# zabaras/deep-turbulence

Measured on AMD Instinct MI355X. Metric: flow-field samples/sec (fwd+log-det+bwd), 64x256x256x4; optimizer step: HipAdam (one-launch Adam, same update as torch.optim.Adam), higher is better.
Workload: dtype f32; 1 GPU; tmglow M: sample()+logdet+backward+Adam, out 256x256x4, L=4, K=16, batch 64/GPU; global_batch=64, parallelism=dp1, world_size_observed=1, rank0_device=AMD Radeon Graphics cuda:0, mix_precision=f32, launch=eager

## Files before the change

deep-turbulence_amd/csrc/tmg_common.h:

```cpp
#pragma once
#include <hip/hip_runtime.h>
#include <stdint.h>
#include <stdlib.h>
#include <atomic>

typedef float f32x4 __attribute__((ext_vector_type(4)));

__device__ __forceinline__ __amdgpu_buffer_rsrc_t tmg_make_rsrc(const void* base, unsigned bytes) {
    return __builtin_amdgcn_make_buffer_rsrc(const_cast<void*>(base), 0, (int)bytes, 0x00020000);
}
__device__ __forceinline__ float4 tmg_bload4(__amdgpu_buffer_rsrc_t rs, unsigned voff, unsigned soff) {
    const f32x4 v = __builtin_bit_cast(f32x4, __builtin_amdgcn_raw_buffer_load_b128(rs, (int)voff, (int)soff, 0));
    return make_float4(v[0], v[1], v[2], v[3]);
}

#define TMG_MAX_IN_SEG 3
#define TMG_MAX_OUT_SEG 3

struct TmgSeg {
    const float* p;
    int stride;
    int off;
    int n;
};
struct TmgOSeg {
    float* p;
    int stride;
    int off;
    int n;
};

__device__ __forceinline__ float wave_sum(float v) {
#pragma unroll
    for (int o = 32; o > 0; o >>= 1) v += __shfl_xor(v, o, 64);
    return v;
}

__device__ __forceinline__ float block_sum_256(float v, float* red ) {
    v = wave_sum(v);
    const int lane = threadIdx.x & 63, w = threadIdx.x >> 6;
    __syncthreads();
    if (lane == 0) red[w] = v;
    __syncthreads();
    return red[0] + red[1] + red[2] + red[3];
}

__device__ __forceinline__ float out_scale_of(const float* kappa) {
    if (!kappa) return 1.0f;
    float k = *kappa;
    k = fminf(fmaxf(k, -4.0f), 1.3862943611198906f);
    return expf(k);
}

#define TMG_PICK_SEG(PTYPE_, ARR, C_, PTR_, STRIDE_, OFF_)                                                \
    PTYPE_ PTR_ = ARR[0].p;                                                                               \
    int STRIDE_ = ARR[0].stride, OFF_ = ARR[0].off;                                                       \
    if (C_ >= ARR[0].n) {                                                                                 \
        C_ -= ARR[0].n; PTR_ = ARR[1].p; STRIDE_ = ARR[1].stride; OFF_ = ARR[1].off;                      \
        if (C_ >= ARR[1].n) { C_ -= ARR[1].n; PTR_ = ARR[2].p; STRIDE_ = ARR[2].stride; OFF_ = ARR[2].off; } \
    }
#define TMG_PICK_OSEG(ARR, NL_, PTR_, STRIDE_, OFF_) TMG_PICK_SEG(float*, ARR, NL_, PTR_, STRIDE_, OFF_)

template <typename P>
__device__ __forceinline__ float4 load_in4(const P& p, int b, int iy, int ix, int c) {
    float4 v = make_float4(0.f, 0.f, 0.f, 0.f);
    if (p.pad_rep) {
        iy = min(max(iy, 0), p.Hin - 1);
        ix = min(max(ix, 0), p.Win - 1);
    } else if (iy < 0 || iy >= p.Hin || ix < 0 || ix >= p.Win) {
        return v;
    }
    if (c >= p.Cin) return v;
    const size_t pix = ((size_t)b * p.Hin + iy) * p.Win + ix;
    if (p.vec4) {
        int cl = c;
        TMG_PICK_SEG(const float*, p.in, cl, sp, ss, so)
        v = *reinterpret_cast<const float4*>(sp + pix * ss + so + cl);
    } else {
        float t[4];
#pragma unroll
        for (int e = 0; e < 4; ++e) {
            int cl = c + e;
            float x = 0.f;
            if (cl < p.Cin) {
                TMG_PICK_SEG(const float*, p.in, cl, sp, ss, so)
                x = sp[pix * ss + so + cl];
            }
            t[e] = x;
        }
        v = make_float4(t[0], t[1], t[2], t[3]);
    }
    if (p.in_scale) {
        float* f = reinterpret_cast<float*>(&v);
#pragma unroll
        for (int e = 0; e < 4; ++e)
            if (c + e < p.Cin) f[e] = f[e] * p.in_scale[c + e] + p.in_shift[c + e];
    }
    if (p.relu_in) {
        v.x = fmaxf(v.x, 0.f);
        v.y = fmaxf(v.y, 0.f);
// ... 248 lines not shown
```

deep-turbulence_amd/csrc/tmg_conv.hip:

```cpp
#include "tmg_common.h"
#include <stdlib.h>

static __device__ float g_tmg_zero_page[64];

struct ConvP {
    TmgSeg in[TMG_MAX_IN_SEG];
    int nseg;
    int vec4;
    int B, Hin, Win, Hout, Wout;
    int ksize, stride;
    int Cin, Cin_pad, Cout, Cout_pad;
    const float* wpk;
    const float* bias;
    const float* kappa;
    const float* in_scale;
    const float* in_shift;
    int relu_in, pad_rep, relu_out, accumulate;
    TmgOSeg out[TMG_MAX_OUT_SEG];
    int nout;
    TmgSeg add;
    int TW_log2, TH;
    int KCH;
    int tiles_x, tiles_y;
    int ntiles, nchunks;
// ... 808 lines not shown
        __syncthreads();
    }
#undef TMG_WG_MFMA
#undef TMG_SB
#undef TMG_WG_ISSUE
#undef TMG_WG_COMMIT
#undef TMG_WG_ISSUE_F
#undef TMG_WG_COMMIT_F
#undef TMG_WG_PATCH_ITEM
#undef TMG_WG_ORIGIN

    const int nws = ksplit ? 1 : 4;
    for (int half = 4; half >= nws; half >>= 1) {
        __syncthreads();
        if (wave >= half && wave < 2 * half) {
            float4* dst = reinterpret_cast<float4*>(lds) + ((wave - half) * NP * NCO) * 64 + lane;
#pragma unroll
            for (int j = 0; j < NP; ++j)
#pragma unroll
                for (int n = 0; n < NCO; ++n)
                    dst[(j * NCO + n) * 64] = make_float4(acc[j][n][0], acc[j][n][1], acc[j][n][2], acc[j][n][3]);
        }
        __syncthreads();
        if (wave < half) {
            const float4* src = reinterpret_cast<const float4*>(lds) + (wave * NP * NCO) * 64 + lane;
#pragma unroll
            for (int j = 0; j < NP; ++j)
#pragma unroll
                for (int n = 0; n < NCO; ++n) {
                    const float4 v = src[(j * NCO + n) * 64];
                    acc[j][n][0] += v.x; acc[j][n][1] += v.y; acc[j][n][2] += v.z; acc[j][n][3] += v.w;
                }
        }
    }
    float bsum = 0.f;
    const bool do_bias = p.dbias && blockIdx.z == 0;
    if (do_bias) {
        __syncthreads();
        *reinterpret_cast<float4*>(lds + tid * 4) = bacc;
        __syncthreads();
        if (tid < NCO * 16) {
            const int c4 = tid >> 2, e = tid & 3;
            for (int t = c4; t < NT; t += NCO * 4) bsum += lds[t * 4 + e];
        }
    }
    if (p.ws) {
        const size_t bl = ((size_t)blockIdx.x * gridDim.y + blockIdx.y) * gridDim.z + blockIdx.z;
        if (wave < nws) {
            float4* slab = reinterpret_cast<float4*>(p.ws) + ((bl * nws + wave) * NP * NCO) * 64 + lane;
#pragma unroll
            for (int j = 0; j < NP; ++j)
#pragma unroll
                for (int n = 0; n < NCO; ++n)
                    slab[(j * NCO + n) * 64] = make_float4(acc[j][n][0], acc[j][n][1], acc[j][n][2], acc[j][n][3]);
        }
        if (do_bias && tid < NCO * 16) {
            float* wsb = p.ws + (size_t)gridDim.x * gridDim.y * gridDim.z * nws * NP * NCO * 256;
            wsb[((size_t)blockIdx.x * gridDim.y + blockIdx.y) * 64 + tid] = bsum;
        }
        return;
    }
    if (wave >= nws) return;
    const float osc = out_scale_of(p.kappa);
#pragma unroll
    for (int j = 0; j < NP; ++j) {
        const int pid = ksplit ? j : w4 + 4 * j;
        if (pid >= npairs) continue;
        const int citg = (pair0 + pid) / ntaps, tap = pair0 + pid - citg * ntaps;
#pragma unroll
        for (int n = 0; n < NCO; ++n) {
            const int co = co0 + n * 16 + li;
            if (co >= p.Cout) continue;
#pragma unroll
            for (int r = 0; r < 4; ++r) {
                const int ci = citg * 16 + q * 4 + r;
                if (ci < p.cin_valid)
                    atomicAdd(p.dW + ((size_t)co * p.cin_dst + ci + (ci < p.ci_split ? p.ci_off0 : p.ci_off1)) * ntaps + tap, acc[j][n][r] * osc);
            }
        }
    }
    if (do_bias && tid < NCO * 16 && co0 + tid < p.Cout) atomicAdd(p.dbias + co0 + tid, bsum * osc);
}

__global__ void conv_wgrad_reduce_kernel(const float* __restrict__ ws, float* __restrict__ dW, float* __restrict__ dbias,
                                         const float* __restrict__ kappa, int gx, int gy, int gz, int NP, int NCO, int PPG,
                                         int pairs_total, int Cin, int Cout, int ntaps, int xchunk, int cin_valid, int ci_split,
                                         int ci_off0, int ci_off1, int ksplit, int bpg, long long dw_gstride, int db_gstride) {
    const int nws = ksplit ? 1 : 4;
    const int items = gy * gz * nws * NP * NCO * 64;
    const int i = blockIdx.x * blockDim.x + threadIdx.x;
    const int x0 = blockIdx.y * xchunk, x1 = min(gx, x0 + xchunk);
    const float osc = out_scale_of(kappa);
    if (i < items) {
        int r_ = i;
        const int lane = r_ & 63; r_ >>= 6;
        const int n = r_ % NCO; r_ /= NCO;
        const int j = r_ % NP; r_ /= NP;
        const int wave = r_ % nws; r_ /= nws;
        const int z = r_ % gz;
        const int y = r_ / gz;
        const int pid = ksplit ? j : wave + 4 * j;
        if (pid < min(PPG, pairs_total - z * PPG)) {
            const size_t per_x = (size_t)gy * gz * nws * NP * NCO * 64;
            const float4* src = reinterpret_cast<const float4*>(ws) + (((((size_t)y * gz + z) * nws + wave) * NP + j) * NCO + n) * 64 + lane;
            float4 a = make_float4(0.f, 0.f, 0.f, 0.f);
            for (int xb = x0; xb < x1; xb += 8) {
                float4 v[8];
#pragma unroll
                for (int u = 0; u < 8; ++u) v[u] = src[(size_t)min(xb + u, x1 - 1) * per_x];
#pragma unroll
                for (int u = 0; u < 8; ++u) {
                    const float wgt = (xb + u < x1) ? 1.f : 0.f;
                    a.x += wgt * v[u].x; a.y += wgt * v[u].y; a.z += wgt * v[u].z; a.w += wgt * v[u].w;
                }
            }
            const int citg = (z * PPG + pid) / ntaps, tap = z * PPG + pid - citg * ntaps;
            const int grp = y / bpg;
            const int co = ((y - grp * bpg) * NCO + n) * 16 + (lane & 15);
            const int ci = citg * 16 + (lane >> 4) * 4;
            dW += (size_t)grp * dw_gstride;
            if (co < Cout) {
                const float av[4] = {a.x, a.y, a.z, a.w};
#pragma unroll
                for (int r = 0; r < 4; ++r)
                    if (ci + r < cin_valid)
                        atomicAdd(dW + ((size_t)co * Cin + ci + r + (ci + r < ci_split ? ci_off0 : ci_off1)) * ntaps + tap, av[r] * osc);
            }
        }
    }
    if (dbias && i < gy * 64) {
        const int y = i >> 6, t = i & 63;
        const int grp = y / bpg;
        const int co = (y - grp * bpg) * NCO * 16 + t;
        dbias += (size_t)grp * db_gstride;
        if (t < NCO * 16 && co < Cout) {
            const float* wsb = ws + (size_t)gx * gy * gz * nws * NP * NCO * 256;
            float a = 0.f;
            for (int xb = x0; xb < x1; xb += 8) {
                float v[8];
#pragma unroll
                for (int u = 0; u < 8; ++u) v[u] = wsb[((size_t)min(xb + u, x1 - 1) * gy + y) * 64 + t];
#pragma unroll
                for (int u = 0; u < 8; ++u) a += (xb + u < x1) ? v[u] : 0.f;
            }
            atomicAdd(dbias + co, a * osc);
        }
    }
}

__global__ void conv_pack_kernel(const float* __restrict__ w, float* __restrict__ wpk, int Cout, int Cin, int ntaps,
                                 int Kpad, int Npad, int mode, int cvalid, int csplit, int cgap, size_t w_bstride, size_t wpk_bstride) {
    w += blockIdx.y * w_bstride;
    wpk += blockIdx.y * wpk_bstride;
    const size_t total = (size_t)ntaps * Kpad * Npad;
    for (size_t i = blockIdx.x * (size_t)blockDim.x + threadIdx.x; i < total; i += (size_t)gridDim.x * blockDim.x) {
        const int c16 = i & 15;
        size_t r = i >> 4;
        const int n = r % Npad;
        r /= Npad;
        const int kb = r % (Kpad >> 4);
        const int tap = r / (Kpad >> 4);
        const int k = kb * 16 + c16;
        float v = 0.f;
        if (mode == 0) {
            if (k < cvalid && n < Cout) v = w[((size_t)n * Cin + k + (k < csplit ? 0 : cgap)) * ntaps + tap];
        } else {
            if (k < Cout && n < cvalid) v = w[((size_t)k * Cin + n + (n < csplit ? 0 : cgap)) * ntaps + (ntaps - 1 - tap)];
        }
        wpk[i] = v;
    }
}

struct PackJob {
    const float* w; float* wpk;
    int Cout, Cin, ntaps, Kpad, Npad, mode, cvalid, csplit, cgap;
};
constexpr int TMG_PACK_JOBS = 48;
struct PackJobs { PackJob j[TMG_PACK_JOBS]; };

__global__ void conv_pack_many_kernel(PackJobs J) {
    const PackJob& jb = J.j[blockIdx.y];
    const float* __restrict__ w = jb.w;
    float* __restrict__ wpk = jb.wpk;
    const int Cout = jb.Cout, Cin = jb.Cin, ntaps = jb.ntaps, Kpad = jb.Kpad, Npad = jb.Npad, mode = jb.mode;
    const int cvalid = jb.cvalid, csplit = jb.csplit, cgap = jb.cgap;
    const size_t total = (size_t)ntaps * Kpad * Npad;
    for (size_t i = blockIdx.x * (size_t)blockDim.x + threadIdx.x; i < total; i += (size_t)gridDim.x * blockDim.x) {
        const int c16 = i & 15;
        size_t r = i >> 4;
        const int n = r % Npad;
        r /= Npad;
        const int kb = r % (Kpad >> 4);
        const int tap = r / (Kpad >> 4);
        const int k = kb * 16 + c16;
        float v = 0.f;
        if (mode == 0) {
            if (k < cvalid && n < Cout) v = w[((size_t)n * Cin + k + (k < csplit ? 0 : cgap)) * ntaps + tap];
        } else {
            if (k < Cout && n < cvalid) v = w[((size_t)k * Cin + n + (n < csplit ? 0 : cgap)) * ntaps + (ntaps - 1 - tap)];
        }
        wpk[i] = v;
    }
}

struct BorderP {
    const float* dy;
    int dy_stride, dy_off, Cdy;
    const float* wpk;
    int Cx, Npad, KB, dy_vec;
    const float* kappa;
    int B, H, W;
    TmgOSeg out[TMG_MAX_OUT_SEG];
    int nborder;
};

__device__ __forceinline__ void border_pixel(int idx, int H, int W, int* y, int* x) {
    if (idx < W) { *y = 0; *x = idx; return; }
    idx -= W;
    if (H > 1) {
        if (idx < W) { *y = H - 1; *x = idx; return; }
        idx -= W;
    }
    const int rows = H - 2;
    if (idx < rows) { *y = 1 + idx; *x = 0; return; }
    idx -= rows;
    *y = 1 + idx; *x = W - 1;
}

__global__ void conv_rep_border_fix_kernel(BorderP p) {
    const size_t total = (size_t)p.B * p.nborder * p.Cx;
// ... 576 lines not shown
    auto fits = [&](int cg, int nc) {
        if (cg > 8) return false;
        const int k4p = cg <= 1 ? 4 : (cg <= 2 ? 8 : (cg <= 4 ? 16 : 32));
        return PH * PW * k4p <= 7 * 512 && 2 * ((size_t)(PH * PW * 16 + 16) * cg + (size_t)(pl->MPIX * 16 + 16) * nc) * 4 <= 160 * 1024;
    };
    int CITG = 1, NCO = 1, bestg = -1;
    for (auto& c : pref) {
        int cg = c[0], nc = c[1];
        if (ntaps == 1) cg *= 4;
        if (cg > cit) {
            if (cit <= 2 && cot >= 8 && nc < 4 && ntaps == 9) continue;
            cg = cit;
        }
        if (nc > cot || (nc == 4 && !allow4)) continue;
        while (cg > 1 && !fits(cg, nc)) --cg;
        if (!fits(cg, nc)) continue;
        const int g = ((cit + cg - 1) / cg) * ((cot + nc - 1) / nc);
        if (g >= gmin) { CITG = cg; NCO = nc; bestg = g; break; }
        if (g > bestg) { CITG = cg; NCO = nc; bestg = g; }
    }
    if (bestg < 0) return -6;
    const int ngroups = (cit + CITG - 1) / CITG;
    pl->CITG = (cit + ngroups - 1) / ngroups;
    pl->NCO = NCO;
    pl->ksplit = ntaps * pl->CITG <= (NCO == 4 ? 5 : 9);
    pl->PPG = ntaps * pl->CITG;
    if (!pl->ksplit && ngroups > 1) {
        const int tp = ntaps * cit, ppg = (((tp + ngroups - 1) / ngroups) + 3) & ~3;
        int span = 0;
        for (int g = 0; g * ppg < tp; ++g) {
            const int a = g * ppg, b = (a + ppg < tp ? a + ppg : tp) - 1;
            if (b / ntaps - a / ntaps + 1 > span) span = b / ntaps - a / ntaps + 1;
        }
        if (ppg < pl->PPG && (ngroups - 1) * ppg < tp && span <= 4 && fits(span, NCO)) { pl->PPG = ppg; pl->CITG = span; }
    }
    const int np = pl->ksplit ? pl->PPG : (pl->PPG + 3) / 4;
    pl->NP = np <= 3 ? 3 : (np <= 5 ? 5 : (np <= 7 ? 7 : (np <= 8 ? 8 : 9)));
    if (pl->NP == 8 && NCO == 4) pl->NP = 9;
    if (np > 9) return -7;
    pl->gy = (cot + NCO - 1) / NCO;
    pl->gz = ngroups;
    int PHe = PH, PWe = PW;
    if (pl->ksplit && NCO == 1 && stride == 1 && TW >= 16 && pl->MPIX == 128) {
        const int k4p = pl->CITG <= 1 ? 4 : (pl->CITG <= 2 ? 8 : (pl->CITG <= 4 ? 16 : 32));
        for (int mp = 512; mp > 128; mp >>= 1) {
            const int th = mp >> twl, ph = th + 2 * halo;
            const int tiles = B * ((Wout + TW - 1) / TW) * ((Hout + th - 1) / th);
            if (ph * PW * k4p <= 7 * 512 && 2 * ((size_t)(ph * PW * 16 + 16) * pl->CITG + (size_t)(mp * 16 + 16) * NCO) * 4 <= 160 * 1024 &&
                tiles >= 4 * tmg_num_cus() / (pl->gy * pl->gz)) {
                pl->MPIX = mp; pl->TH = th;
                pl->tiles_y = (Hout + th - 1) / th;
                pl->ntiles = tiles;
                PHe = ph;
                break;
            }
        }
    }
    pl->lds_bytes = 2 * ((size_t)(PHe * PWe * 16 + 16) * pl->CITG + (size_t)(pl->MPIX * 16 + 16) * NCO) * 4;
    if (pl->lds_bytes < 8192) pl->lds_bytes = 8192;
    if (pl->lds_bytes < (size_t)4 * pl->NP * NCO * 1024) pl->lds_bytes = (size_t)4 * pl->NP * NCO * 1024;
    int gx = tmg_num_cus() / (pl->gy * ngroups);
    if (gx > pl->ntiles / 4) gx = pl->ntiles / 4;
    if (gx < 1) gx = 1;
    pl->gx = gx;
    pl->ws_floats = (size_t)gx * pl->gy * pl->gz * (pl->ksplit ? 1 : 4) * pl->NP * NCO * 256 + (size_t)gx * pl->gy * 64;
    return 0;
}

static int plan_wgrad(int B, int Hout, int Wout, int ksize, int stride, int Cin, int Cout, WgradPlan* pl) {
    const int rc = plan_wgrad_impl(B, Hout, Wout, ksize, stride, Cin, Cout, pl, true);
    if (rc == 0 && pl->NP == 5 && pl->NCO == 4) return plan_wgrad_impl(B, Hout, Wout, ksize, stride, Cin, Cout, pl, false);
    return rc;
}

extern "C" int64_t tmg_conv_wgrad_ws_floats(const int64_t* dims) {
    WgradPlan pl;
    if (plan_wgrad((int)dims[0], (int)dims[3], (int)dims[4], (int)dims[5], (int)dims[6], (int)dims[7], (int)dims[8], &pl) != 0) return 0;
    return (int64_t)pl.ws_floats;
}

static int wgrad_impl(const void* const* in_ptrs, const int64_t* in_desc, int64_t nseg, const void* in_scale,
                      const void* in_shift, const void* dy, const int64_t* dy_desc, void* dW, void* dbias,
                      const void* kappa, void* ws, int64_t ws_floats, const int64_t* dims, hipStream_t st,
                      const long long* gtab, int ngroups, int dy_goff, long long dw_gstride, int db_gstride, int64_t* plan = nullptr) {
    WgradP p;
    p.nseg = (int)nseg;
    p.vec4 = tmg_decode_in(p.in, in_ptrs, in_desc, nseg).vec4;
    p.B = (int)dims[0]; p.Hin = (int)dims[1]; p.Win = (int)dims[2]; p.Hout = (int)dims[3]; p.Wout = (int)dims[4];
    p.ksize = (int)dims[5]; p.stride = (int)dims[6]; p.Cin = (int)dims[7]; p.Cout = (int)dims[8];
    p.relu_in = (int)dims[9]; p.pad_rep = (int)dims[10];
    p.cin_dst = dims[11] > 0 ? (int)dims[11] : p.Cin;
    p.cin_valid = dims[12] > 0 ? (int)dims[12] : (p.cin_dst < p.Cin ? p.cin_dst : p.Cin);
    p.ci_split = dims[13] > 0 ? (int)dims[13] : 0x7fffffff;
    p.ci_off0 = (int)dims[14]; p.ci_off1 = (int)dims[15];
    if (p.ksize != 1 && p.ksize != 3) return -2;
    p.Cin_pad = (p.Cin + 15) & ~15;
    p.in_scale = (const float*)in_scale; p.in_shift = (const float*)in_shift;
    p.dy = TmgSeg{(const float*)dy, (int)dy_desc[0], (int)dy_desc[1], p.Cout};
    p.dy_vec4 = (((p.dy.stride | p.dy.off) & 3) == 0) && ((((uintptr_t)dy) & 15) == 0);
    p.dW = (float*)dW; p.dbias = (float*)dbias; p.kappa = (const float*)kappa;
    WgradPlan pl;
    const int rc = plan_wgrad(p.B, p.Hout, p.Wout, p.ksize, p.stride, p.Cin, p.Cout, &pl);
    if (rc != 0) return rc;
    p.TW_log2 = pl.twl; p.TH = pl.TH; p.MPIX = pl.MPIX; p.tiles_x = pl.tiles_x; p.tiles_y = pl.tiles_y; p.ntiles = pl.ntiles; p.CITG = pl.CITG;
    p.PPG = pl.PPG;
    const int bpg = pl.gy;
    if (ngroups > 1) {
        pl.gy = bpg * ngroups;
        int gx = tmg_num_cus() / (pl.gy * pl.gz);
        if (gx > pl.ntiles / 4) gx = pl.ntiles / 4;
        if (gx < 1) gx = 1;
        pl.gx = gx;
        pl.ws_floats = (size_t)gx * pl.gy * pl.gz * (pl.ksplit ? 1 : 4) * pl.NP * pl.NCO * 256 + (size_t)gx * pl.gy * 64;
    }
    p.ws = (ws && (size_t)ws_floats >= pl.ws_floats && (((uintptr_t)ws) & 15) == 0) ? (float*)ws : nullptr;
    dim3 grid(pl.gx, pl.gy, pl.gz);
    p.ksplit = pl.ksplit;
    p.gtab = gtab; p.bpg = bpg; p.dy_goff = dy_goff; p.dw_gstride = dw_gstride; p.db_gstride = db_gstride;
    p.fstage = p.vec4 && p.dy_vec4 && (p.Cout % 4 == 0) && (p.Cin % 4 == 0) && (long)p.Hin * p.Win < (1 << 24) && (long)p.Hout * p.Wout < (1 << 24);
    for (int i = 0; i < p.nseg; ++i)
        if (p.in[i].stride >= (1 << 24) || (long)p.B * p.Hin * p.Win * p.in[i].stride >= (1L << 31)) p.fstage = 0;
    if (p.dy.stride >= (1 << 24) || (long)p.B * p.Hout * p.Wout * p.dy.stride >= (1L << 31)) p.fstage = 0;
    if (ngroups > 1 && (!p.fstage || !p.ws)) return -100;
    int lrc = -7;
#define TMG_WG_CASE(NP_, NCO_)                                                                    \
    if (pl.NP == NP_ && pl.NCO == NCO_)                                                           \
        lrc = p.fstage ? launch_wgrad<NP_, NCO_, true>(p, grid, pl.lds_bytes, st, plan, pl.ws_floats)                       \
                       : launch_wgrad<NP_, NCO_, false>(p, grid, pl.lds_bytes, st, plan, pl.ws_floats);
    TMG_WG_CASE(3, 1) TMG_WG_CASE(3, 2) TMG_WG_CASE(3, 4)
    TMG_WG_CASE(5, 1) TMG_WG_CASE(5, 2)
    TMG_WG_CASE(7, 1) TMG_WG_CASE(7, 2)
    TMG_WG_CASE(8, 1) TMG_WG_CASE(8, 2)
    TMG_WG_CASE(9, 1) TMG_WG_CASE(9, 2)
#undef TMG_WG_CASE
    if (lrc != 0 || plan) return lrc;
    if (p.ws) {
        const int items = pl.gy * pl.gz * (pl.ksplit ? 1 : 4) * pl.NP * pl.NCO * 64;
        int xchunk = 32;
        const int xc = (pl.gx + xchunk - 1) / xchunk;
        hipLaunchKernelGGL(conv_wgrad_reduce_kernel, dim3((items + 255) / 256, xc), dim3(256), 0, st, (const float*)p.ws, p.dW, p.dbias,
                           p.kappa, pl.gx, pl.gy, pl.gz, pl.NP, pl.NCO, pl.PPG, (p.Cin_pad >> 4) * p.ksize * p.ksize, p.cin_dst, p.Cout, p.ksize * p.ksize, xchunk,
                           p.cin_valid, p.ci_split, p.ci_off0, p.ci_off1, pl.ksplit, bpg, dw_gstride, db_gstride);
        TMG_CHECK_LAUNCH();
    }
    return 0;
}

extern "C" int tmg_conv_wgrad(const void* const* in_ptrs, const int64_t* in_desc, int64_t nseg, const void* in_scale,
                              const void* in_shift, const void* dy, const int64_t* dy_desc, void* dW, void* dbias,
                              const void* kappa, void* ws, int64_t ws_floats, const int64_t* dims, hipStream_t st) {
    return wgrad_impl(in_ptrs, in_desc, nseg, in_scale, in_shift, dy, dy_desc, dW, dbias, kappa, ws, ws_floats, dims, st, nullptr, 1, 0, 0, 0);
}

extern "C" int tmg_conv_wgrad_plan(const void* const* in_ptrs, const int64_t* in_desc, int64_t nseg, const void* in_scale,
                                   const void* in_shift, const void* dy, const int64_t* dy_desc, void* dW, void* dbias,
                                   const void* kappa, void* ws, int64_t ws_floats, const int64_t* dims, hipStream_t st, int64_t ngroups,
                                   int64_t* plan) {
    if (!plan || ngroups < 1) return -3;
    for (int i = 0; i < 15; ++i) plan[i] = -1;
    return wgrad_impl(in_ptrs, in_desc, nseg, in_scale, in_shift, dy, dy_desc, dW, dbias, kappa, ws, ws_floats, dims, st, nullptr,
                      (int)ngroups, 0, 0, 0, plan);
}

extern "C" int tmg_conv_wgrad_grouped(const void* const* in_ptrs, const int64_t* in_desc, int64_t nseg, const void* gtab,
                                      int64_t ngroups, const int64_t* gdims, const void* dy, const int64_t* dy_desc, void* dW,
                                      void* dbias, void* ws, int64_t ws_floats, const int64_t* dims, hipStream_t st) {
    if (ngroups < 1 || !gtab) return -3;
    return wgrad_impl(in_ptrs, in_desc, nseg, nullptr, nullptr, dy, dy_desc, dW, dbias, nullptr, ws, ws_floats, dims, st,
                      (const long long*)gtab, (int)ngroups, (int)gdims[0], (long long)gdims[1], (int)gdims[2]);
}

extern "C" int64_t tmg_conv_wgrad_grouped_ws_floats(const int64_t* dims, int64_t ngroups) {
    WgradPlan pl;
    if (plan_wgrad((int)dims[0], (int)dims[3], (int)dims[4], (int)dims[5], (int)dims[6], (int)dims[7], (int)dims[8], &pl) != 0) return 0;
    const int gy = pl.gy * (int)ngroups;
    int gx = tmg_num_cus() / (gy * pl.gz);
    if (gx > pl.ntiles / 4) gx = pl.ntiles / 4;
    if (gx < 1) gx = 1;
    return (int64_t)((size_t)gx * gy * pl.gz * (pl.ksplit ? 1 : 4) * pl.NP * pl.NCO * 256 + (size_t)gx * gy * 64);
}

template <int NT>
static int launch_border_mfma(const BorderMP& m, int blocks, hipStream_t st, int64_t* plan) {
    if (plan) {
        const int64_t v[5] = {1, NT, m.ksplit, m.tile0[16], blocks};
        for (int i = 0; i < 5; ++i) plan[i] = v[i];
        return 0;
    }
    hipLaunchKernelGGL(conv_rep_border_mfma_kernel<NT>, dim3(blocks), dim3(256), 0, st, m);
    TMG_CHECK_LAUNCH();
    return 0;
}

static int rep_border_impl(const void* dy, const int64_t* dy_desc, const void* w, const void* kappa, void* const* out_ptrs,
                           const int64_t* out_desc, int64_t nout, const int64_t* dims, hipStream_t st, int64_t* plan) {
    BorderP p;
    p.dy = (const float*)dy; p.dy_stride = (int)dy_desc[0]; p.dy_off = (int)dy_desc[1];
    p.B = (int)dims[0]; p.H = (int)dims[1]; p.W = (int)dims[2]; p.Cdy = (int)dims[3]; p.Cx = (int)dims[4];
    p.wpk = (const float*)w; p.kappa = (const float*)kappa;
    p.Npad = (p.Cx + 15) & ~15;
    p.KB = (p.Cdy + 15) >> 4;
    p.dy_vec = ((p.Cdy & 15) == 0) && (((p.dy_stride | p.dy_off) & 3) == 0) && ((((uintptr_t)dy) & 15) == 0);
    const TmgSegList so = tmg_decode_out(p.out, out_ptrs, out_desc, nout);
    if (p.H == 1 && p.W == 1) p.nborder = 1;
    else if (p.H == 1) p.nborder = p.W;
    else p.nborder = 2 * p.W + (p.W > 1 ? 2 : 1) * (p.H - 2);
    bool mf = p.H >= 2 && p.W >= 2 && (p.Cdy & 3) == 0 && (((p.dy_stride | p.dy_off) & 3) == 0) && ((((uintptr_t)dy) & 15) == 0) &&
              (p.Cx & 3) == 0 && p.Npad <= 128 && so.vec4;
    if (mf) {
        BorderMP m;
        m.b = p;
        const int cnt[8] = {p.H - 2, p.H - 2, p.W - 2, p.W - 2, 1, 1, 1, 1};
        int t0 = 0;
        for (int v = 0; v < 16; ++v) {
            const int c = v < 4 ? v : 4 + (v - 4) / 3;
            m.cnt[c] = cnt[c] > 0 ? cnt[c] : 1;
            m.tile0[v] = t0;
            t0 += cnt[c] > 0 ? (p.B * cnt[c] + 15) / 16 : 0;
        }
        m.tile0[16] = t0;
        int S = (4096 + t0 - 1) / t0;
        if (S > p.KB / 4) S = p.KB / 4;
        if (S < 1) S = 1;
        m.ksplit = S;
        const long items = (long)t0 * S;
        const int blocks = (int)((items + 3) / 4 < 4096 ? (items + 3) / 4 : 4096);
        switch (p.Npad >> 4) {
            case 1: return launch_border_mfma<1>(m, blocks, st, plan);
            case 2: return launch_border_mfma<2>(m, blocks, st, plan);
            case 3: return launch_border_mfma<3>(m, blocks, st, plan);
            case 4: return launch_border_mfma<4>(m, blocks, st, plan);
            case 5: return launch_border_mfma<5>(m, blocks, st, plan);
            case 6: return launch_border_mfma<6>(m, blocks, st, plan);
            case 7: return launch_border_mfma<7>(m, blocks, st, plan);
            default: return launch_border_mfma<8>(m, blocks, st, plan);
        }
    }
    const size_t total = (size_t)p.B * p.nborder * p.Cx;
    const int blocks = (int)((total + 255) / 256 < 4096 ? (total + 255) / 256 : 4096);
    if (plan) {
        const int64_t v[5] = {0, 0, 1, 0, blocks};
        for (int i = 0; i < 5; ++i) plan[i] = v[i];
        return 0;
    }
    hipLaunchKernelGGL(conv_rep_border_fix_kernel, dim3(blocks), dim3(256), 0, st, p);
    TMG_CHECK_LAUNCH();
    return 0;
}

extern "C" int tmg_conv_rep_border_fix(const void* dy, const int64_t* dy_desc, const void* w, const void* kappa,
                                       void* const* out_ptrs, const int64_t* out_desc, int64_t nout, const int64_t* dims,
                                       hipStream_t st) {
// ... 22 lines not shown
```

deep-turbulence_amd/csrc/tmg_wino.hip:

```cpp
#include "tmg_common.h"
#include <stdlib.h>
#include <type_traits>

struct WinoP {
    TmgSeg in[TMG_MAX_IN_SEG];
    int nseg;
    int B, Hin, Win;
    int Cin, Cin_pad, Cout, Npad;
    const float* U;
    const float* bias;
    int relu_in, pad_rep;
    TmgOSeg out[TMG_MAX_OUT_SEG];
    int tiles_x, tiles_y, ntiles;
    int nchunks;
};

__global__ void wino_pack_kernel(const float* __restrict__ w, float* __restrict__ U, int Cout, int Cin, int K, int N, int Kpad, int Npad, int mode) {
    const size_t total = (size_t)Kpad * Npad;
    for (size_t i = blockIdx.x * (size_t)blockDim.x + threadIdx.x; i < total; i += (size_t)gridDim.x * blockDim.x) {
        const int c16 = i & 15;
        size_t r = i >> 4;
        const int n = r % Npad;
        const int kb = r / Npad;
        const int k = kb * 16 + c16;
// ... 1362 lines not shown
    _Pragma("unroll") for (int s = (S0); s < (S1); ++s) {                                                              \
        __builtin_amdgcn_sched_barrier(0);                                                                             \
        const int sx = ((2 * (s >> 1)) * PW + 8 * (s & 1)) * CSX;           \
        const int sd = ((2 * (s >> 1)) * 16 + 8 * (s & 1)) * CSD;                                                      \
        float xa[2][CIT], dh[2][NCO];                                                                                  \
        _Pragma("unroll") for (int i = 0; i < CIT; ++i) {                                                              \
            const float u0 = fmaf((XRB)[oxb0 + sx + 16 * i], sg, (XRB)[oxa0 + sx + 16 * i]);                           \
            const float u1 = fmaf((XRB)[oxb1 + sx + 16 * i], sg, (XRB)[oxa1 + sx + 16 * i]);                           \
            const float u2 = fmaf((XRB)[oxb2 + sx + 16 * i], sg, (XRB)[oxa2 + sx + 16 * i]);                           \
            xa[0][i] = u0 - u2;                                                                                        \
            xa[1][i] = fmaf(u1, s1, u2);                                                                               \
        }                                                                                                              \
        _Pragma("unroll") for (int n = 0; n < NCO; ++n) {                                                              \
            const float* dp_ = (DRB) + od + sd + 16 * n;                                                               \
            const f2 d_ = k00 * dp_[0] + k01 * dp_[CSD] + k10 * dp_[16 * CSD] + k11 * dp_[17 * CSD];                   \
            dh[0][n] = d_.x; dh[1][n] = d_.y;                                                                          \
        }                                                                                                              \
        __builtin_amdgcn_sched_barrier(0);                                                                             \
        _Pragma("unroll") for (int i = 0; i < CIT; ++i)                                                                \
            _Pragma("unroll") for (int n = 0; n < NCO; ++n) {                                                          \
                acc[0][i][n] = __builtin_amdgcn_mfma_f32_16x16x4f32(xa[0][i], dh[0][n], acc[0][i][n], 0, 0, 0);         \
                acc[1][i][n] = __builtin_amdgcn_mfma_f32_16x16x4f32(xa[1][i], dh[1][n], acc[1][i][n], 0, 0, 0);         \
            }                                                                                                          \
    }
    if constexpr (DB) {
        int cur = 0;
        if ((int)blockIdx.x < p.ntiles) {
            TMG_WW_ISSUE((int)blockIdx.x)
            TMG_WW_COMMIT(XR, DR)
            if ((int)blockIdx.x + G < p.ntiles) TMG_WW_ISSUE((int)blockIdx.x + G)
        }
        __syncthreads();
        for (int tile = blockIdx.x; tile < p.ntiles; tile += G) {
            const float* xrb = XR + cur * BUFW;
            const float* drb = DR + cur * BUFW;
            TMG_WW_KSTEPS(0, 4, xrb, drb)
            __builtin_amdgcn_sched_barrier(0);
            if (tile + G < p.ntiles) {
                TMG_WW_COMMIT(XR + (cur ^ 1) * BUFW, DR + (cur ^ 1) * BUFW)
                if (tile + 2 * G < p.ntiles) TMG_WW_ISSUE(tile + 2 * G)
            }
            __builtin_amdgcn_sched_barrier(0);
            TMG_WW_KSTEPS(4, 8, xrb, drb)
            __syncthreads();
            cur ^= 1;
        }
    } else {
        if ((int)blockIdx.x < p.ntiles) TMG_WW_ISSUE((int)blockIdx.x)
        for (int tile = blockIdx.x; tile < p.ntiles; tile += G) {
            TMG_WW_COMMIT(XR, DR)
            __syncthreads();
            if (tile + G < p.ntiles) TMG_WW_ISSUE(tile + G)
            TMG_WW_KSTEPS(0, 8, XR, DR)
            __syncthreads();
        }
    }
#undef TMG_WW_COMMIT
#undef TMG_WW_KSTEPS
#undef TMG_WW_ISSUE
    const size_t bl = ((size_t)blockIdx.x * gridDim.y + blockIdx.y) * gridDim.z + blockIdx.z;
    float4* slab = reinterpret_cast<float4*>(p.ws) + ((bl * 8 + wave) * (2 * CIT * NCO)) * 64 + lane;
#pragma unroll
    for (int e = 0; e < 2; ++e)
#pragma unroll
        for (int i = 0; i < CIT; ++i)
#pragma unroll
            for (int n = 0; n < NCO; ++n)
                slab[((e * CIT + i) * NCO + n) * 64] = make_float4(acc[e][i][n][0], acc[e][i][n][1], acc[e][i][n][2], acc[e][i][n][3]);
    if (p.want_bias && blockIdx.z == 0) {
        __syncthreads();
        *reinterpret_cast<float4*>(lds + tid * 4) = bacc;
        __syncthreads();
        if (tid < NCO * 16) {
            const int c4 = tid >> 2, e = tid & 3;
            float bs = 0.f;
            for (int t = c4; t < NT; t += KD) bs += lds[t * 4 + e];
            float* wsb = p.ws + (size_t)gridDim.x * gridDim.y * gridDim.z * 8 * (2 * CIT * NCO) * 256;
            wsb[((size_t)blockIdx.x * gridDim.y + blockIdx.y) * 64 + tid] = bs;
        }
    }
}

template <int NG>
__global__ __launch_bounds__(64 * NG) TMG_PACKED_F32 void wino_wgrad_reduce_kernel(const float* __restrict__ ws, float* __restrict__ dW, float* __restrict__ dbias,
                                                                   int gx, int gy, int gz, int CIT, int NCO, int Cin, int Cout, int cin_dst,
                                                                   int cin_valid, int ci_split, int ci_off0, int ci_off1, int bpg,
                                                                   long long dw_gstride, int db_gstride) {
    extern __shared__ __attribute__((aligned(16))) float red_[];
    float (*red)[64][37] = reinterpret_cast<float (*)[64][37]>(red_);
    const int lane = threadIdx.x & 63, grp = threadIdx.x >> 6;
    int r_ = blockIdx.x;
    const int n = r_ % NCO; r_ /= NCO;
    const int i = r_ % CIT; r_ /= CIT;
    const int bz = r_ % gz, by = r_ / gz;
    const int li = lane & 15, q = lane >> 4;
    float4 m[16];
#pragma unroll
    for (int pz = 0; pz < 16; ++pz) m[pz] = make_float4(0.f, 0.f, 0.f, 0.f);
    for (int bx = grp; bx < gx; bx += NG) {
        const size_t bl = ((size_t)bx * gy + by) * gz + bz;
#pragma unroll
        for (int pz = 0; pz < 16; ++pz) {
            const int w = pz >> 1, e = pz & 1;
            const float4 v = reinterpret_cast<const float4*>(ws)[((bl * 8 + w) * (2 * CIT * NCO) + (e * CIT + i) * NCO + n) * 64 + lane];
            m[pz].x += v.x; m[pz].y += v.y; m[pz].z += v.z; m[pz].w += v.w;
        }
    }
    float tap[4][9];
#pragma unroll
    for (int r = 0; r < 4; ++r) {
        float M[4][4];
#pragma unroll
        for (int a = 0; a < 4; ++a)
#pragma unroll
            for (int b = 0; b < 4; ++b) {
                const float4 v = m[a * 4 + b];
                M[a][b] = r == 0 ? v.x : (r == 1 ? v.y : (r == 2 ? v.z : v.w));
            }
        float T[3][4];
#pragma unroll
        for (int b = 0; b < 4; ++b) {
            T[0][b] = M[0][b] + M[1][b] + M[2][b];
            T[1][b] = M[1][b] - M[2][b];
            T[2][b] = M[1][b] + M[2][b] - M[3][b];
        }
#pragma unroll
        for (int a = 0; a < 3; ++a) {
            tap[r][a * 3 + 0] = T[a][0] + T[a][1] + T[a][2];
            tap[r][a * 3 + 1] = T[a][1] - T[a][2];
            tap[r][a * 3 + 2] = T[a][1] + T[a][2] - T[a][3];
        }
    }
    if (grp > 0) {
#pragma unroll
        for (int r = 0; r < 4; ++r)
#pragma unroll
            for (int k = 0; k < 9; ++k) red[grp - 1][lane][r * 9 + k] = tap[r][k];
    }
    __syncthreads();
    const int group = by / bpg, cb = by - group * bpg;
    dW += (size_t)group * dw_gstride;
    if (grp == 0) {
        const int co = (cb * NCO + n) * 16 + li;
#pragma unroll
        for (int r = 0; r < 4; ++r) {
            const int ci = (bz * CIT + i) * 16 + 4 * q + r;
            if (co >= Cout || ci >= Cin || ci >= cin_valid) continue;
            float* dst = dW + ((size_t)co * cin_dst + ci + (ci < ci_split ? ci_off0 : ci_off1)) * 9;
#pragma unroll
            for (int k = 0; k < 9; ++k) {
                float v = tap[r][k];
#pragma unroll
                for (int g_ = 0; g_ < NG - 1; ++g_) v += red[g_][lane][r * 9 + k];
                dst[k] += v;
            }
        }
    }
    if (dbias && bz == 0 && i == 0 && n == 0 && threadIdx.x < NCO * 16) {
        dbias += (size_t)group * db_gstride;
        const int c = threadIdx.x, co = cb * NCO * 16 + c;
        if (co < Cout) {
            const float* wsb = ws + (size_t)gx * gy * gz * 8 * (2 * CIT * NCO) * 256;
            float s_ = 0.f;
            for (int bx = 0; bx < gx; ++bx) s_ += wsb[((size_t)bx * gy + by) * 64 + c];
            dbias[co] += s_;
        }
    }
}

struct WinoWPlan { int CIT, NCO, gx, gy, gz; size_t ws_floats; };

static int plan_wino_wgrad(int B, int H, int W, int Cin, int Cout, int ngroups, WinoWPlan* pl) {
    const int cit = (Cin + 15) >> 4, cot = (Cout + 15) >> 4;
    if (cit < 2 || cot < 2) return -100;
    pl->gz = (cit + 3) / 4;
    const int citg = (cit + pl->gz - 1) / pl->gz;
    pl->CIT = citg <= 2 ? 2 : (citg == 3 ? 3 : 4);
    pl->gy = (cot + 3) / 4;
    const int cotg = (cot + pl->gy - 1) / pl->gy;
    pl->NCO = cotg <= 2 ? 2 : (cotg == 3 ? 3 : 4);
    pl->gy *= ngroups;
    const int ntiles = B * ((W + 15) / 16) * ((H + 7) / 8);
    int gx = tmg_num_cus() / (pl->gy * pl->gz);
    if (gx > ntiles / 2) gx = ntiles / 2;
    if (gx < 1) gx = 1;
    pl->gx = gx;
    pl->ws_floats = (size_t)gx * pl->gy * pl->gz * 8 * (2 * pl->CIT * pl->NCO) * 256 + (size_t)gx * pl->gy * 64;
    return 0;
}

extern "C" int64_t tmg_conv_wino_wgrad_ws_floats(const int64_t* dims) {
    WinoWPlan pl;
    if (plan_wino_wgrad((int)dims[0], (int)dims[1], (int)dims[2], (int)dims[3], (int)dims[4], 1, &pl) != 0) return 0;
    return (int64_t)pl.ws_floats;
}

static inline int wino_wgrad_reduce_groups(int gx) { return gx >= 64 ? 16 : (gx >= 32 ? 8 : 4); }

#define TMG_WINO_WG_PLAN_N 11
template <int CIT, int NCO>
static int launch_wino_wgrad(const WinoWP& p, const WinoWPlan& pl, hipStream_t st, int64_t* plan) {
    constexpr size_t one = (size_t)(180 * (CIT * 16 + 8) + 128 * (NCO * 16 + 8)) * sizeof(float);
    constexpr bool DB = 2 * one <= 160 * 1024;
    if (plan) {
        const int64_t v[TMG_WINO_WG_PLAN_N] = {CIT, NCO, DB ? 1 : 0, pl.gx, pl.gy, pl.gz, p.bpg, wino_wgrad_reduce_groups(pl.gx), p.ntiles,
                                               (int64_t)(DB ? 2 * one : (one < 8192 ? 8192 : one)), (int64_t)pl.ws_floats};
        for (int i = 0; i < TMG_WINO_WG_PLAN_N; ++i) plan[i] = v[i];
        return 0;
    }
    const double ngr = p.gtab ? (double)(pl.gy / (p.bpg > 0 ? p.bpg : 1)) : 1.0;
    TmgProf prof(TMG_PROF_WINO_WG, ngr * 2.0 * p.B * p.Hin * p.Win * (double)p.Cout * p.Cin * 9, st);
    const size_t lds = DB ? 2 * one : (one < 8192 ? 8192 : one);
    TMG_LDS_OPTIN((&wino_wgrad_kernel<CIT, NCO, DB>));
    hipLaunchKernelGGL((wino_wgrad_kernel<CIT, NCO, DB>), dim3(pl.gx, pl.gy, pl.gz), dim3(512), lds, st, p);
    TMG_CHECK_LAUNCH();
    return 0;
}

static int wino_wgrad_impl(const void* const* in_ptrs, const int64_t* in_desc, int64_t nseg, const void* dy, const int64_t* dy_desc,
                           void* dW, void* dbias, void* ws, int64_t ws_floats, const int64_t* dims, hipStream_t st, const long long* gtab,
                           int ngroups, int dy_goff, long long dw_gstride, int db_gstride, int64_t* plan = nullptr) {
    WinoWP p;
    p.nseg = (int)nseg;
    if (p.nseg < 1 || p.nseg > TMG_MAX_IN_SEG) return -3;
    const TmgSegList si = tmg_decode_in(p.in, in_ptrs, in_desc, nseg);
    bool ok = si.vec4;
    p.B = (int)dims[0]; p.Hin = (int)dims[1]; p.Win = (int)dims[2]; p.Cin = (int)dims[3]; p.Cout = (int)dims[4];
    p.relu_in = (int)dims[5]; p.pad_rep = (int)dims[6];
    const int cin_dst = dims[7] > 0 ? (int)dims[7] : p.Cin;
    const int cin_valid = dims[8] > 0 ? (int)dims[8] : (cin_dst < p.Cin ? cin_dst : p.Cin);
    const int ci_split = dims[9] > 0 ? (int)dims[9] : 0x7fffffff;
    const int ci_off0 = (int)dims[10], ci_off1 = (int)dims[11];
    if (si.csum != p.Cin) return -3;
    p.dy = (const float*)dy; p.dy_stride = (int)dy_desc[0]; p.dy_off = (int)dy_desc[1];
    if (((p.dy_stride | p.dy_off | dy_goff) & 3) || (((uintptr_t)dy) & 15) || (p.Cin & 3) || (p.Cout & 3)) ok = false;
    WinoWPlan pl;
    if (!ok || plan_wino_wgrad(p.B, p.Hin, p.Win, p.Cin, p.Cout, ngroups, &pl) != 0) return -100;
    if (!ws || (size_t)ws_floats < pl.ws_floats || (((uintptr_t)ws) & 15)) return -100;
    p.ws = (float*)ws;
    p.want_bias = dbias ? 1 : 0;
    p.gtab = gtab; p.bpg = pl.gy / ngroups; p.dy_goff = dy_goff;
    p.tiles_x = (p.Win + 15) / 16; p.tiles_y = (p.Hin + 7) / 8;
    p.ntiles = p.B * p.tiles_x * p.tiles_y;
    if (p.ntiles <= 0) return 0;
    if ((long long)p.B * p.Hin * p.Win >= (1LL << 31)) return -100;
    int rc = -7;
#define TMG_WW_CASE(C_, N_) if (pl.CIT == C_ && pl.NCO == N_) rc = launch_wino_wgrad<C_, N_>(p, pl, st, plan);
    TMG_WW_CASE(2, 2) TMG_WW_CASE(2, 3) TMG_WW_CASE(2, 4) TMG_WW_CASE(3, 2) TMG_WW_CASE(3, 3) TMG_WW_CASE(3, 4) TMG_WW_CASE(4, 2) TMG_WW_CASE(4, 3)
    TMG_WW_CASE(4, 4)
#undef TMG_WW_CASE
    if (rc != 0 || plan) return rc;
    const int ng = wino_wgrad_reduce_groups(pl.gx);
    if (ng == 16) {
        TMG_LDS_OPTIN((&wino_wgrad_reduce_kernel<16>));
        hipLaunchKernelGGL(wino_wgrad_reduce_kernel<16>, dim3(pl.gy * pl.gz * pl.CIT * pl.NCO), dim3(1024), 15 * 64 * 37 * sizeof(float), st,
                           (const float*)p.ws, (float*)dW, (float*)dbias, pl.gx, pl.gy, pl.gz, pl.CIT, pl.NCO, p.Cin, p.Cout, cin_dst, cin_valid,
                           ci_split, ci_off0, ci_off1, p.bpg, dw_gstride, db_gstride);
    } else if (ng == 8) {
        TMG_LDS_OPTIN((&wino_wgrad_reduce_kernel<8>));
        hipLaunchKernelGGL(wino_wgrad_reduce_kernel<8>, dim3(pl.gy * pl.gz * pl.CIT * pl.NCO), dim3(512), 7 * 64 * 37 * sizeof(float), st,
                           (const float*)p.ws, (float*)dW, (float*)dbias, pl.gx, pl.gy, pl.gz, pl.CIT, pl.NCO, p.Cin, p.Cout, cin_dst, cin_valid,
                           ci_split, ci_off0, ci_off1, p.bpg, dw_gstride, db_gstride);
    } else {
        hipLaunchKernelGGL(wino_wgrad_reduce_kernel<4>, dim3(pl.gy * pl.gz * pl.CIT * pl.NCO), dim3(256), 3 * 64 * 37 * sizeof(float), st,
                           (const float*)p.ws, (float*)dW, (float*)dbias, pl.gx, pl.gy, pl.gz, pl.CIT, pl.NCO, p.Cin, p.Cout, cin_dst, cin_valid,
                           ci_split, ci_off0, ci_off1, p.bpg, dw_gstride, db_gstride);
    }
    TMG_CHECK_LAUNCH();
    return 0;
}

extern "C" int tmg_conv_wino_wgrad(const void* const* in_ptrs, const int64_t* in_desc, int64_t nseg, const void* dy, const int64_t* dy_desc,
                                   void* dW, void* dbias, void* ws, int64_t ws_floats, const int64_t* dims, hipStream_t st) {
    return wino_wgrad_impl(in_ptrs, in_desc, nseg, dy, dy_desc, dW, dbias, ws, ws_floats, dims, st, nullptr, 1, 0, 0, 0);
}

extern "C" int tmg_conv_wino_wgrad_grouped(const void* const* in_ptrs, const int64_t* in_desc, int64_t nseg, const void* gtab, int64_t ngroups,
                                           const int64_t* gdims, const void* dy, const int64_t* dy_desc, void* dW, void* dbias, void* ws,
                                           int64_t ws_floats, const int64_t* dims, hipStream_t st) {
    if (ngroups < 1 || !gtab) return -3;
    return wino_wgrad_impl(in_ptrs, in_desc, nseg, dy, dy_desc, dW, dbias, ws, ws_floats, dims, st, (const long long*)gtab, (int)ngroups,
                           (int)gdims[0], (long long)gdims[1], (int)gdims[2]);
}

extern "C" int tmg_conv_wino_wgrad_plan(const void* const* in_ptrs, const int64_t* in_desc, int64_t nseg, const void* dy, const int64_t* dy_desc,
                                        void* dW, void* dbias, void* ws, int64_t ws_floats, const int64_t* dims, hipStream_t st, int64_t ngroups,
                                        int64_t* plan) {
    if (!plan || ngroups < 1) return -3;
    for (int i = 0; i < TMG_WINO_WG_PLAN_N; ++i) plan[i] = -1;
    return wino_wgrad_impl(in_ptrs, in_desc, nseg, dy, dy_desc, dW, dbias, ws, ws_floats, dims, st, nullptr, (int)ngroups, 0, 0, 0, plan);
}

extern "C" int64_t tmg_conv_wino_wgrad_grouped_ws_floats(const int64_t* dims, int64_t ngroups) {
    WinoWPlan pl;
    if (plan_wino_wgrad((int)dims[0], (int)dims[1], (int)dims[2], (int)dims[3], (int)dims[4], (int)ngroups, &pl) != 0) return 0;
    return (int64_t)pl.ws_floats;
}
```

deep-turbulence_amd/tmg_hip.py:

```python
import ctypes
import os
import weakref
import subprocess
import sys

import torch

_HERE = os.path.dirname(os.path.abspath(__file__))
LIB_PATH = os.path.join(_HERE, "libtmglow_hip.so")
CSRC = os.path.join(_HERE, "csrc")
SOURCES = ["tmg_conv.hip", "tmg_pointwise.hip", "tmg_physics.hip", "tmg_mix16.hip", "tmg_coupling.hip", "tmg_wino.hip", "tmg_thin.hip", "tmg_glue.hip", "tmg_ensemble.hip", "tmg_spectrum.hip", "tmg_scores.hip", "tmg_tspec.hip", "tmg_quant.hip", "tmg_gram.hip", "tmg_sfun.hip"]
NO_PACKED_F32 = ["tmg_wino.hip", "tmg_conv.hip", "tmg_coupling.hip", "tmg_thin.hip", "tmg_mix16.hip", "tmg_spectrum.hip", "tmg_tspec.hip"]
_lib = None

c_i64 = ctypes.c_int64
c_vp = ctypes.c_void_p

EXPORTS = [
    "tmg_conv_pack", "tmg_conv_pack_map", "tmg_conv_fwd", "tmg_conv_fwd_add", "tmg_affine_bwd_scaled", "tmg_c1_fwd_add", "tmg_conv_wgrad", "tmg_conv_wgrad_ws_floats", "tmg_conv_rep_border_fix", "tmg_conv_dgrad_direct",
    "tmg_affine_apply", "tmg_affine_apply_pass", "tmg_bn_finalize", "tmg_affine_bwd", "tmg_lstm_pointwise_fwd", "tmg_lstm_pointwise_bwd", "tmg_gauss_fwd",
    "tmg_gauss_bwd", "tmg_checker", "tmg_upsample_fwd", "tmg_upsample_bwd", "tmg_chan_reduce", "tmg_bn_bwd_apply",
    "tmg_phys_fwd", "tmg_phys_rms", "tmg_phys_bwd", "tmg_conv_wgrad_grouped", "tmg_conv_wgrad_grouped_ws_floats", "tmg_conv_pack_batched", "tmg_masked_add", "tmg_c1x2_fwd", "tmg_c1_fwd", "tmg_c1_bwd", "tmg_dense2_bwd", "tmg_dkappa", "tmg_prof_enable", "tmg_prof_collect", "tmg_mix_f16", "tmg_phys_bwd_dev", "tmg_coupling_fwd", "tmg_coupling_bwd",
    "tmg_conv_wino_pack", "tmg_conv_wino_fwd", "tmg_conv_wino_narrow", "tmg_conv_wino_wgrad", "tmg_conv_wino_wgrad_ws_floats", "tmg_mix_f32", "tmg_lu_fold_fwd", "tmg_lu_fold_bwd", "tmg_lu_fold_bwd_split", "tmg_level_finish", "tmg_conv_wgrad_thin_grouped", "tmg_mix_wgrad_grouped", "tmg_layer_planes", "tmg_conv_wino_wgrad_grouped", "tmg_conv_wino_wgrad_grouped_ws_floats", "tmg_adam_step", "tmg_chan_moments", "tmg_bn_finalize64", "tmg_mix_f32_affine_fwd", "tmg_mix_f32_affine_bwd", "tmg_conv_pack_many", "tmg_pad_halves", "tmg_coupling_fwd_halves", "tmg_coupling_bwd_halves", "tmg_fill_i64", "tmg_conv_wino_pack3", "tmg_conv_wino_fwd3", "tmg_mat_inverse", "tmg_gauss_sample", "tmg_reverse_loss_fwd", "tmg_reverse_loss_bwd", "tmg_sum_terms", "tmg_vec_sum", "tmg_level_pack", "tmg_spread2", "tmg_phys_fields", "tmg_phys_fields_bwd",
    "tmg_gauss_sample_keyed", "tmg_ens_accum", "tmg_ens_time_finalize", "tmg_ens_turb_accum", "tmg_ens_turb_finalize",
    "tmg_spec_rows", "tmg_spec_cols", "tmg_spec_accum", "tmg_spec_finalize",
    "tmg_ens_score_store", "tmg_ens_score_step",
]
PLAN_EXPORTS = ["tmg_conv_fwd_plan", "tmg_conv_wgrad_plan", "tmg_conv_rep_border_plan", "tmg_conv_wino_fwd_plan", "tmg_conv_wino_fwd3_plan",
                "tmg_conv_wino_narrow_plan", "tmg_conv_wino_wgrad_plan", "tmg_c1x2_fwd_plan", "tmg_c1_fwd_plan",
                "tmg_conv_wgrad_thin_grouped_plan", "tmg_mix_wgrad_grouped_plan"]
TSPEC_EXPORTS = ["tmg_tspec_store", "tmg_tspec_block", "tmg_tspec_finalize"]
QUANT_EXPORTS = ["tmg_ens_quant_step"]
GRAM_EXPORTS = ["tmg_ens_gram_plan", "tmg_ens_gram_step", "tmg_ens_gram_traj"]
SFUN_EXPORTS = ["tmg_ens_sfun_plan", "tmg_ens_sfun_step"]
RET_I64 = ("tmg_conv_wgrad_ws_floats", "tmg_conv_wgrad_grouped_ws_floats", "tmg_conv_wino_wgrad_ws_floats",
           "tmg_conv_wino_wgrad_grouped_ws_floats")


def build(force=False, verbose=False):
    from concurrent.futures import ThreadPoolExecutor
    inc = os.path.join(os.path.dirname(_HERE), "include")
    headers = [os.path.join(CSRC, "tmg_common.h"), os.path.join(inc, "tmglow_hip.h"), os.path.join(inc, "tmglow_hip_plan.h"),
               os.path.join(inc, "tmglow_hip_tspec.h"), os.path.join(inc, "tmglow_hip_quant.h"),
               os.path.join(inc, "tmglow_hip_gram.h"), os.path.join(inc, "tmglow_hip_sfun.h")]
    hmt = max(os.path.getmtime(h) for h in headers)
    objdir = os.path.join(_HERE, "build")
    os.makedirs(objdir, exist_ok=True)
    hipcc = os.environ.get("HIPCC", "/opt/rocm/bin/hipcc")
    flags = ["--offload-arch=gfx950", "-O3", "-fPIC", "-std=c++17", "-Wno-unused-result", "-I", inc]
    jobs, objs, stamps = [], [], []
    for src in SOURCES:
        sp, ob = os.path.join(CSRC, src), os.path.join(objdir, src.replace(".hip", ".o"))
        objs.append(ob)
        extra = ["-Xclang", "-target-feature", "-Xclang", "-packed-fp32-ops"] if src in NO_PACKED_F32 else []
        line = " ".join(flags + extra)
        stamp = ob + ".flags"
        old = open(stamp).read() if os.path.exists(stamp) else None
        if force or old != line or not os.path.exists(ob) or os.path.getmtime(ob) < max(os.path.getmtime(sp), hmt):
            jobs.append([hipcc] + flags + extra + ["-c", sp, "-o", ob])
            stamps.append((stamp, line))
    if not jobs and os.path.exists(LIB_PATH) and all(os.path.getmtime(LIB_PATH) >= os.path.getmtime(o) for o in objs):
        return LIB_PATH

    def run(cmd):
        if verbose:
            print(" ".join(cmd), flush=True)
        r = subprocess.run(cmd, stderr=subprocess.PIPE, text=True)
        err = "\n".join(ln for ln in r.stderr.splitlines() if "'-packed-fp32-ops' is not a recognized feature" not in ln)
        if err.strip():
            print(err, file=sys.stderr, flush=True)
        if r.returncode != 0:
            raise subprocess.CalledProcessError(r.returncode, cmd)

    with ThreadPoolExecutor(max_workers=4) as ex:
        list(ex.map(run, jobs))
    for stamp, line in stamps:
        open(stamp, "w").write(line)
    run([hipcc, "--offload-arch=gfx950", "-shared", "-fPIC"] + objs + ["-o", LIB_PATH])
    return LIB_PATH


def lib():
    global _lib
    if _lib is None:
        if not os.path.exists(LIB_PATH):
            raise RuntimeError("libtmglow_hip.so is missing (%s): run `python -c 'import __graft_entry__ as g; g.build()'`. "
                               "There is no fallback path." % LIB_PATH)
        _lib = ctypes.CDLL(LIB_PATH)
        for name in EXPORTS:
            getattr(_lib, name).restype = c_i64 if name in RET_I64 else ctypes.c_int
        _lib.tmg_prof_name.restype = ctypes.c_char_p
        for name in PLAN_EXPORTS:
            getattr(_lib, name).restype = ctypes.c_int
            getattr(_lib, name).argtypes = PLAN_ARGTYPES[name]
        for name in TSPEC_EXPORTS + QUANT_EXPORTS + GRAM_EXPORTS + SFUN_EXPORTS:
            getattr(_lib, name).restype = ctypes.c_int
    return _lib


def prof_enable(on):
    lib().tmg_prof_enable(c_i64(int(on)))


def prof_kernel_id(name):
    l = lib()
    for k in range(64):
        if l.tmg_prof_name(c_i64(k)).decode() == name:
            return k
    raise KeyError(name)


def prof_collect():
    l = lib()
    nk = 64
    buf = (ctypes.c_double * (3 * nk))()
    n = l.tmg_prof_collect(buf, c_i64(nk))
    out = {}
    for k in range(n):
        if buf[3 * k] > 0:
            out[l.tmg_prof_name(c_i64(k)).decode()] = (int(buf[3 * k]), buf[3 * k + 1], buf[3 * k + 2])
    return out


def _stream():
    return c_vp(torch._C._cuda_getCurrentRawStream(torch._C._cuda_getDevice()))


def _chk(code, name):
    if code != 0:
        raise RuntimeError("%s failed with code %d" % (name, code))


def _ptr(t):
    return c_vp(t.data_ptr()) if t is not None else c_vp(0)


def check_act(t):
    if not (t.is_cuda and t.dtype == torch.float32):
        raise RuntimeError("TM-Glow HIP ops need fp32 tensors on a HIP device (got %s on %s); there is no CPU path"
                           % (t.dtype, t.device))


def seg(t):
    check_act(t)
    B, H, W, C = t.shape
    s = t.stride()
    ps = s[2] if W > 1 else (s[1] // W if H > 1 else (s[0] // (H * W) if B > 1 else C))
    ok = s[3] == 1 or C == 1
    if W > 1:
        ok = ok and (H == 1 or s[1] == W * ps) and (B == 1 or s[0] == H * W * ps)
    if not ok or ps < C:
        raise RuntimeError("tensor is not an NHWC channel-slice: shape %s strides %s" % (tuple(t.shape), s))
    return (t.data_ptr(), int(ps), 0, int(C))


def check_device(t):
    if t.is_cuda and t.device.index != torch.cuda.current_device():
        raise RuntimeError("TM-Glow HIP op called with a tensor on %s while the current device is cuda:%d: wrap the call in "
                           "`with torch.cuda.device(t.device):` (or torch.cuda.set_device once per process)"
                           % (t.device, torch.cuda.current_device()))


def nhwc(x):
    check_act(x)
    check_device(x)
    return x.permute(0, 2, 3, 1).contiguous()


def nchw(t):
    return t.permute(0, 3, 1, 2)


def _segs(tensors):
    d = [seg(t) for t in tensors]
    ptrs = (c_vp * len(d))(*[x[0] for x in d])
    desc = (c_i64 * (3 * len(d)))(*[v for x in d for v in (x[1], x[2], x[3])])
    return ptrs, desc, len(d)

# ... 152 lines not shown
    _chk(lib().tmg_conv_wino_pack(_ptr(w), _ptr(U), c_i64(Cout), c_i64(Cin), c_i64(mode), c_i64(nvalid), _stream()), "tmg_conv_wino_pack")
    return U


_WINO_PRECISION = ["bf16x3" if os.environ.get("TMG_WINO_BF3") else "f32"]


def set_winograd_precision(kind):
    if kind not in ("f32", "bf16x3"):
        raise ValueError("Winograd precision must be 'f32' or 'bf16x3', got %r" % (kind,))
    _WINO_PRECISION[0] = kind


def winograd_precision():
    return _WINO_PRECISION[0]


def conv_wino_pack3(w, mode=0, nvalid=0):
    Cout, Cin = w.shape[0], w.shape[1]
    assert w.shape[2] == 3 and w.shape[3] == 3
    w = w.contiguous()
    K, N = (Cin, Cout) if mode == 0 else (Cout, nvalid if 0 < nvalid < Cin else Cin)
    U = torch.empty(16 * ((K + 31) // 32 * 32) * ((N + 15) // 16 * 16) * 3, device=w.device, dtype=torch.int16)
    _chk(lib().tmg_conv_wino_pack3(_ptr(w), _ptr(U), c_i64(Cout), c_i64(Cin), c_i64(mode), c_i64(nvalid), _stream()), "tmg_conv_wino_pack3")
    return U


def _wino_fwd(name, inputs, U, Cout, outs, bias, *flags):
    if isinstance(outs, torch.Tensor):
        outs = [outs]
    B, Hin, Win, _ = inputs[0].shape
    ip, idesc, n_in = _segs(inputs)
    op, odesc, n_out = _segs(outs)
    Cin = sum(t.shape[3] for t in inputs)
    assert sum(t.shape[3] for t in outs) == Cout and outs[0].shape[1] == Hin and outs[0].shape[2] == Win
    return _launched(getattr(lib(), name)(ip, idesc, c_i64(n_in), _ptr(U), _ptr(bias), op, odesc, c_i64(n_out),
                                          _i64(B, Hin, Win, Cin, Cout, *flags), _stream()), name)


def conv_wino_fwd3(inputs, U, Cout, outs, bias=None, relu_in=False, pad_rep=False):
    return _wino_fwd("tmg_conv_wino_fwd3", inputs, U, Cout, outs, bias, relu_in, pad_rep)


def conv_wino_narrow(inputs, U, Cout, outs, bias=None, relu_in=False, pad_rep=False, relu_out=False):
    return _wino_fwd("tmg_conv_wino_narrow", inputs, U, Cout, outs, bias, relu_in, pad_rep, relu_out)


def conv_wino_fwd(inputs, U, Cout, outs, bias=None, relu_in=False, pad_rep=False):
    return _wino_fwd("tmg_conv_wino_fwd", inputs, U, Cout, outs, bias, relu_in, pad_rep)


def conv3x3_auto(inputs, weight, Cout, outs, bias=None, relu_in=False, pad_rep=False, relu_out=False, dgrad=False, nvalid=0):
    Cin = sum(t.shape[3] for t in inputs)
    mode = 1 if dgrad else 0
    if not relu_out and wino_eligible(Cin, Cout, 3, 1):
        if (_WINO_PRECISION[0] == "bf16x3"
                and conv_wino_fwd3(inputs, conv_wino_pack3(weight, mode, nvalid), Cout, outs, bias=bias, relu_in=relu_in, pad_rep=pad_rep)):
            return None
        if conv_wino_fwd(inputs, conv_wino_pack(weight, mode, nvalid), Cout, outs, bias=bias, relu_in=relu_in, pad_rep=pad_rep):
            return None
    if wino_narrow_eligible(Cin, Cout):
        if conv_wino_narrow(inputs, conv_wino_pack(weight, mode, nvalid), Cout, outs, bias=bias, relu_in=relu_in, pad_rep=pad_rep,
                            relu_out=relu_out):
            return None
    wpk = conv_pack(weight, mode, nvalid, (nvalid, 1 << 30, 0)) if (dgrad and nvalid) else conv_pack(weight, mode)
    conv_fwd(inputs, wpk, Cout, 3, 1, outs, bias=bias, relu_in=relu_in, pad_rep=pad_rep, relu_out=relu_out)
    return wpk


_WS = {}


def workspace(nfloats, device):
    if torch.cuda.is_current_stream_capturing():
        return torch.empty(max(int(nfloats), 1), device=device, dtype=torch.float32)
    key = (device.index, torch._C._cuda_getCurrentRawStream(torch._C._cuda_getDevice()))
    buf = _WS.get(key)
    if buf is None or buf.numel() < nfloats:
        buf = torch.empty(max(int(nfloats), 1 << 20), device=device, dtype=torch.float32)
        _WS[key] = buf
    return buf


_WINO_WGRAD_CIN_MIN = 32
_WINO_WGRAD_PIX_MIN = 1 << 20


def conv_wgrad(inputs, dy, dW, dbias, ksize, stride, kappa=None, in_scale=None, in_shift=None, relu_in=False, pad_rep=False,
               use_ws=True, cin_dst=0, cin_valid=0, ci_split=0, ci_off0=0, ci_off1=0):
    B, Hin, Win, _ = inputs[0].shape
    _, Hout, Wout, Cout = dy.shape
    ip, idesc, n_in = _segs(inputs)
    Cin = sum(t.shape[3] for t in inputs)
    if (ksize == 3 and stride == 1 and kappa is None and in_scale is None and use_ws and Cin >= 32
            and (Cout >= 128 or (Cout >= 32 and Cin >= _WINO_WGRAD_CIN_MIN and B * Hin * Win >= _WINO_WGRAD_PIX_MIN))
            and conv_wino_wgrad(inputs, dy, dW, dbias, relu_in, pad_rep, cin_dst, cin_valid, ci_split, ci_off0, ci_off1)):
        return
    dims = _i64(B, Hin, Win, Hout, Wout, ksize, stride, Cin, Cout, relu_in, pad_rep, cin_dst, cin_valid, ci_split, ci_off0, ci_off1)
    ws = workspace(lib().tmg_conv_wgrad_ws_floats(dims), dy.device) if use_ws else None
    _chk(lib().tmg_conv_wgrad(ip, idesc, c_i64(n_in), _ptr(in_scale), _ptr(in_shift), _ptr(dy), _d2(dy), _ptr(dW), _ptr(dbias),
                              _ptr(kappa), _ptr(ws), c_i64(ws.numel() if ws is not None else 0), dims, _stream()), "tmg_conv_wgrad")


def wino_wgrad_eligible(Cin, Cout):
    return Cin >= 32 and Cout >= 128


def conv_wino_wgrad(inputs, dy, dW, dbias, relu_in=False, pad_rep=False, cin_dst=0, cin_valid=0, ci_split=0, ci_off0=0, ci_off1=0):
    B, Hin, Win, _ = inputs[0].shape
    Cout = dy.shape[3]
    ip, idesc, n_in = _segs(inputs)
    Cin = sum(t.shape[3] for t in inputs)
    wd = _i64(B, Hin, Win, Cin, Cout, relu_in, pad_rep, cin_dst, cin_valid, ci_split, ci_off0, ci_off1)
    need = lib().tmg_conv_wino_wgrad_ws_floats(wd)
    if need > 0:
        ws = workspace(need, dy.device)
        rc = lib().tmg_conv_wino_wgrad(ip, idesc, c_i64(n_in), _ptr(dy), _d2(dy), _ptr(dW), _ptr(dbias), _ptr(ws), c_i64(ws.numel()), wd, _stream())
        if _launched(rc, "tmg_conv_wino_wgrad"):
            return True
    return False


_GTAB = {}


def _segment_table(rows, device):
    flat = [int(v) for r in rows for v in r]
    if torch.cuda.is_current_stream_capturing():
        t = torch.empty((len(rows), len(rows[0])), dtype=torch.int64, device=device)
        _chk(lib().tmg_fill_i64(_ptr(t), _i64(*flat), c_i64(len(flat)), _stream()), "tmg_fill_i64")
        return t
    key = (device.index, len(rows), tuple(flat))
    t = _GTAB.get(key)
    if t is None:
        if len(_GTAB) > 1024:
            _GTAB.clear()
        t = torch.empty((len(rows), len(rows[0])), dtype=torch.int64, device=device)
        _chk(lib().tmg_fill_i64(_ptr(t), _i64(*flat), c_i64(len(flat)), _stream()), "tmg_fill_i64")
        _GTAB[key] = t
    return t


def layer_planes(src):
    B, Hh, Ww, CP = src.shape
    assert src.is_contiguous() and CP % 4 == 0
    dst = torch.empty((CP // 2, B, Hh, Ww, 2), device=src.device, dtype=torch.float32)
    _chk(lib().tmg_layer_planes(_ptr(src), _ptr(dst), c_i64(B * Hh * Ww), c_i64(CP), _stream()), "tmg_layer_planes")
    return dst


def _pixel_linear(t):
    B, Hh, Ww, _ = t.shape
    return t.stride(3) == 1 and (Hh == 1 or t.stride(1) == t.stride(2) * Ww) and (B == 1 or t.stride(0) == t.stride(2) * Ww * Hh)


def _group_rows(group_inputs, group_dy=None):
    first = group_inputs[0]
    n_in = len(first)
    dy_pairs = group_dy is not None and isinstance(group_dy[0], (tuple, list))
    rows = []
    for segs in group_inputs:
        assert len(segs) == n_in and all(a.shape == b.shape and a.stride(2) % 4 == b.stride(2) % 4 for a, b in zip(segs, first))
        row = []
        for t in segs:
            row += list(seg(t))
        row += [0, 0, 0, 0] * (3 - n_in)
        if group_dy is None:
            row += [0, 0, 0, 0]
        elif dy_pairs:
            a, b = group_dy[len(rows)]
            row += [seg(a)[0], seg(a)[1], seg(b)[0], seg(b)[1]]
        else:
            row += [seg(group_dy[len(rows)])[0], seg(group_dy[len(rows)])[1], 0, 0]
        rows.append(row)
    return rows


def conv_wgrad_thin_grouped(group_inputs, dy, dy_group_channels, dW, relu_in=False, gtab=None):
    first = group_inputs[0]
    B, Hin, Win, _ = first[0].shape
    if not all(t.stride(2) % 4 == 0 and t.data_ptr() % 16 == 0 for segs in group_inputs for t in segs):
        return -100
    if gtab is None:
        gtab = _segment_table(_group_rows(group_inputs), dy.device)
    return lib().tmg_conv_wgrad_thin_grouped(_ptr(gtab), c_i64(len(group_inputs)), _i64(*[t.shape[3] for t in first]), c_i64(len(first)),
                                             _ptr(dy), c_i64(dy.stride(2)), _ptr(dW),
                                             _i64(B, Hin, Win, sum(t.shape[3] for t in first), relu_in, int(dy_group_channels)), _stream())


def mix_wgrad_grouped(group_inputs, group_dy, dW, dbias, gtab=None):
    first = group_inputs[0]
    B, Hin, Win, _ = first[0].shape
    pairs = isinstance(group_dy[0], (tuple, list))
    assert all(_pixel_linear(t) for segs in group_inputs for t in segs)
    assert all(_pixel_linear(t) for e in group_dy for t in (e if pairs else (e,)))
    if gtab is None:
        gtab = _segment_table(_group_rows(group_inputs, group_dy), dW.device)
    return lib().tmg_mix_wgrad_grouped(_ptr(gtab), c_i64(len(group_inputs)), _ptr(dW), _ptr(dbias),
                                       _i64(B * Hin * Win, sum(t.shape[3] for t in first)), _stream())


def conv_wgrad_grouped(group_inputs, dy, dy_group_channels, dW, dbias, ksize, stride, relu_in=False, pad_rep=False, cin_dst=0,
                       cin_valid=0, ci_split=0, ci_off0=0, ci_off1=0, group_dy=None):
    dy_pairs = group_dy is not None and isinstance(group_dy[0], (tuple, list))
    if dy_pairs:
        if not (ksize == 1 and stride == 1 and int(dy_group_channels) in (16, 32) and os.environ.get("TMG_NO_MIX_WGRAD_KERNEL") is None):
            group_dy = [torch.cat(list(t), 3) for t in group_dy]
            dy_pairs = False
    if dy is None:
        dy = group_dy[0][0] if dy_pairs else group_dy[0]
        if dy_pairs:
            assert all(a.shape == dy.shape and b.shape == dy.shape for a, b in group_dy)
        else:
            assert all(t.shape == dy.shape and t.stride() == dy.stride() for t in group_dy)
    G = len(group_inputs)
    first = group_inputs[0]
    B, Hin, Win, _ = first[0].shape
    _, Hout, Wout, _ = dy.shape
    Cg = int(dy_group_channels)
    ip, idesc, n_in = _segs(first)
    Cin = sum(t.shape[3] for t in first)
    gtab = _segment_table(_group_rows(group_inputs, group_dy), dy.device)
    if group_dy is None and ksize == 3 and stride == 1 and Cin >= 20 and Cg >= 32:
        wd = _i64(B, Hin, Win, Cin, Cg, relu_in, pad_rep, cin_dst, cin_valid, ci_split, ci_off0, ci_off1)
        need = lib().tmg_conv_wino_wgrad_grouped_ws_floats(wd, c_i64(G))
        if need > 0:
            ws = workspace(need, dy.device)
            gd = _i64(Cg, dW[0].numel(), dbias[0].numel() if dbias is not None else 0)
            rc = lib().tmg_conv_wino_wgrad_grouped(ip, idesc, c_i64(n_in), _ptr(gtab), c_i64(G), gd, _ptr(dy), _d2(dy), _ptr(dW), _ptr(dbias),
                                                   _ptr(ws), c_i64(ws.numel()), wd, _stream())
            if _launched(rc, "tmg_conv_wino_wgrad_grouped"):
                return True
    if (group_dy is not None and ksize == 1 and stride == 1 and Cg == Cin and Cin in (16, 32) and cin_dst in (0, Cin)
            and cin_valid in (0, Cin) and ci_split == 0 and os.environ.get("TMG_NO_MIX_WGRAD_KERNEL") is None
            and all(_pixel_linear(t) for segs in group_inputs for t in segs)
            and all(_pixel_linear(t) for e in group_dy for t in (e if dy_pairs else (e,)))):
        rc = mix_wgrad_grouped(group_inputs, group_dy, dW, dbias, gtab=gtab)
        if _launched(rc, "tmg_mix_wgrad_grouped"):
            return True
    if dy_pairs:
        return conv_wgrad_grouped(group_inputs, None, dy_group_channels, dW, dbias, ksize, stride, relu_in=relu_in, pad_rep=pad_rep,
                                  cin_dst=cin_dst, cin_valid=cin_valid, ci_split=ci_split, ci_off0=ci_off0, ci_off1=ci_off1,
                                  group_dy=[torch.cat(list(t), 3) for t in group_dy])
    if (group_dy is None and ksize == 3 and stride == 1 and Cg in (2, 4) and dW.shape[1] == 4 and not pad_rep and dbias is None and cin_dst in (0, Cin)
            and cin_valid in (0, Cin) and ci_split == 0 and Cin in (12, 20, 36, 68) and os.environ.get("TMG_NO_THIN_WGRAD") is None
            and all(t.stride(2) % 4 == 0 and t.data_ptr() % 16 == 0 for segs in group_inputs for t in segs)):
        rc = conv_wgrad_thin_grouped(group_inputs, dy, Cg, dW, relu_in=relu_in, gtab=gtab)
        if _launched(rc, "tmg_conv_wgrad_thin_grouped"):
            return True
    dims = _i64(B, Hin, Win, Hout, Wout, ksize, stride, Cin, Cg, relu_in, pad_rep, cin_dst, cin_valid, ci_split, ci_off0, ci_off1)
    ws = workspace(lib().tmg_conv_wgrad_grouped_ws_floats(dims, c_i64(G)), dy.device)
    gd = _i64(Cg, dW[0].numel(), dbias[0].numel() if dbias is not None else 0)
    rc = lib().tmg_conv_wgrad_grouped(ip, idesc, c_i64(n_in), _ptr(gtab), c_i64(G), gd, _ptr(dy), _d2(dy), _ptr(dW), _ptr(dbias),
                                      _ptr(ws), c_i64(ws.numel()), dims, _stream())
    return _launched(rc, "tmg_conv_wgrad_grouped")


def _halves(t):
    if isinstance(t, (tuple, list)):
        a, b = t
        assert a.shape == b.shape
        return a, b
    ch = t.shape[3] // 2
    return t[..., :ch], t[..., ch:]


def coupling_fwd(x, out, rsave, y2save, D, hc, wz, bz, kappa, Wm, bm, logdet, reverse, wz_d1col):
    x1, x2 = _halves(x)
    o1, o2 = _halves(out)
    B, Hh, Ww, ch = x1.shape
    s1, s2, t1, t2, sh = seg(x1), seg(x2), seg(o1), seg(o2), seg(hc)
    assert rsave.is_contiguous() and D.is_contiguous() and (y2save is None or y2save.is_contiguous()) and wz.is_contiguous()
    dims = _i64(B, Hh, Ww, 2 * ch, 1 if reverse else 0, s1[1], t1[1], sh[1], wz.shape[1], wz_d1col, s2[1], t2[1])
    rc = lib().tmg_coupling_fwd_halves(c_vp(s1[0]), c_vp(s2[0]), c_vp(t1[0]), c_vp(t2[0]), _ptr(rsave), _ptr(y2save), _ptr(D), c_vp(sh[0]),
                                       _ptr(wz), _ptr(bz), _ptr(kappa), _ptr(Wm), _ptr(bm), _ptr(logdet), dims, _stream())
    return _launched(rc, "tmg_coupling_fwd_halves")


def coupling_bwd(dout, x2, r, g, Wm, wz, kappa, DH, dtin, G0, GD, wz_d1col, fwd=False):
    d1, d2 = _halves(dout)
    t1, t2 = _halves(dtin)
    B, Hh, Ww, ch = d1.shape
    assert x2.shape[3] == ch
    sd1, sd2, sx, sh, st1, st2 = seg(d1), seg(d2), seg(x2), seg(DH), seg(t1), seg(t2)
    assert r.is_contiguous() and G0.is_contiguous() and GD.is_contiguous() and Wm.is_contiguous() and wz.is_contiguous()
    dims = _i64(B, Hh, Ww, 2 * ch, sd1[1], sx[1], sh[1], st1[1], wz.shape[1], wz_d1col, sd2[1], st2[1], 1 if fwd else 0)
    rc = lib().tmg_coupling_bwd_halves(c_vp(sd1[0]), c_vp(sd2[0]), c_vp(sx[0]), _ptr(r), _ptr(g), _ptr(Wm), _ptr(wz), _ptr(kappa), c_vp(sh[0]),
                                       c_vp(st1[0]), c_vp(st2[0]), _ptr(G0), _ptr(GD), dims, _stream())
    return _launched(rc, "tmg_coupling_bwd_halves")


def mix_f16(x, W, bias, y, transposed=False):
    B, Hh, Ww, C = x.shape
    check_act(W)
    assert W.is_contiguous() and W.shape == (C, C) and y.shape == x.shape
    _chk(lib().tmg_mix_f16(_ptr(x), _d2(x), _ptr(W), _ptr(bias), _ptr(y), _d2(y), _i64(B * Hh * Ww, C, 1 if transposed else 0), _stream()),
         "tmg_mix_f16")


def mat_inverse(W, b=None):
    K, C = W.shape[0], W.shape[1]
    W = W.contiguous()
    Winv = torch.empty_like(W)
    binv = torch.empty((K, C), device=W.device, dtype=torch.float32) if b is not None else None
    _chk(lib().tmg_mat_inverse(_ptr(W), _ptr(b.contiguous() if b is not None else None), _ptr(Winv), _ptr(binv), _i64(K, C), _stream()),
         "tmg_mat_inverse")
    return Winv, binv


def lu_fold_fwd(tab, sign_s, perm, iperm, W, Wm, bm, ld, reverse, sgn, hw):
    K, C = sign_s.shape
    assert W.dtype == torch.float64 and C <= 256
    _chk(lib().tmg_lu_fold_fwd(_ptr(tab), _ptr(sign_s), _ptr(perm), _ptr(iperm), _ptr(W), _ptr(Wm), _ptr(bm), _ptr(ld), _i64(K, C, reverse),
                               _flts([sgn, hw]), _stream()), "tmg_lu_fold_fwd")


def lu_fold_bwd(tab, sign_s, perm, iperm, W, dWm, dbm, dld, dl, du, dlogs, da, db, reverse, sgn, hw, dWm_tail=None, dbm_tail=None):
    K, C = sign_s.shape
    _chk(lib().tmg_lu_fold_bwd_split(_ptr(tab), _ptr(sign_s), _ptr(perm), _ptr(iperm), _ptr(W), _ptr(dWm), _ptr(dbm), _ptr(dWm_tail),
                                     _ptr(dbm_tail), _ptr(dld), _ptr(dl), _ptr(du), _ptr(dlogs), _ptr(da), _ptr(db), _i64(K, C, reverse),
                                     _flts([sgn, hw]), _stream()), "tmg_lu_fold_bwd_split")


def level_finish(Wz, dWz, Bz, dBz, Kp, tmpX, tmpC, dW1, dW2, dK, ws, ch, Cc):
    NL, C = dBz.shape
    for t in (Wz, dWz, Bz, dBz, Kp, tmpX, tmpC, dW1, dW2, dK, ws):
        assert t is None or t.is_contiguous()
    assert ws.numel() >= 4 * NL
    _chk(lib().tmg_level_finish(_ptr(Wz), _ptr(dWz), _ptr(Bz), _ptr(dBz), _ptr(Kp), _ptr(tmpX), _ptr(tmpC), _ptr(dW1), _ptr(dW2), _ptr(dK),
                                _ptr(ws), _i64(NL, C, ch, Cc, tmpC.shape[1] if tmpC is not None else 4), _stream()), "tmg_level_finish")


def adam_step(tab, chunks, nchunks, lr, b1, b2, eps, wd, bc1, bc2s, amsgrad):
    _chk(lib().tmg_adam_step(_ptr(tab), _ptr(chunks), _i64(nchunks, 1 if amsgrad else 0), _flts([lr, b1, b2, eps, wd, bc1, bc2s, 1.0 - b1, 1.0 - b2]), _stream()),
         "tmg_adam_step")
# ... 587 lines not shown
```

deep-turbulence_amd/tmg_ops.py:

```python
import collections
import math
import numbers

import os
import threading
import weakref

import torch

import tmg_hip as H

LOG5 = math.log(5.0)
LOG4 = math.log(4.0)
SPLIT_LIMITS = (-2.0, LOG5, -2.0, LOG5)
TOP_LIMITS = (0.0, 0.0, -10.0, LOG5)


class _ZeroPool:
    CHUNK = 8 << 20
    LIMIT = 2 << 20

    def __init__(self):
        self.lock = threading.Lock()
        self.cur = {}
# ... 279 lines not shown

    @staticmethod
    def forward(ctx, x, gamma, beta, weight, mean, rstd, a, bsh, training):
        x = x if x.stride(3) == 1 else x.contiguous()
        B, Hh, Ww, _ = x.shape
        Cout = weight.shape[0]
        out = empty((B, Hh, Ww, Cout), x.device)
        wpk = H.conv_pack(weight, 0)
        H.conv_fwd([x], wpk, Cout, 3, 1, [out], in_scale=a, in_shift=bsh, relu_in=True)
        ctx.training = training
        ctx.save_for_backward(x, gamma, weight, mean, rstd, a, bsh)
        return out

    @staticmethod
    def backward(ctx, dout):
        x, gamma, weight, mean, rstd, a, bsh = ctx.saved_tensors
        dy = dout.contiguous()
        B, Hh, Ww, C = x.shape
        n = B * Hh * Ww
        dW = zeros_like(weight)
        H.conv_wgrad([x], dy, dW, None, 3, 1, in_scale=a, in_shift=bsh, relu_in=True)
        wpk_t = H.conv_pack(weight, 1)
        G = empty((B, Hh, Ww, C), x.device)
        H.conv_fwd([dy], wpk_t, C, 3, 1, [G])
        s = zeros((3, C), x.device)
        s0, s1 = s[0], s[1]
        H.chan_reduce(x, G, a, bsh, mean, rstd, s0, s1, 1)
        dgamma, dbeta = s1, s0
        dx = empty((B, Hh, Ww, C), x.device)
        if ctx.training:
            H.bn_bwd_apply(x, G, a, bsh, mean, rstd, gamma, s0, s1, dx, False, divisor=n)
        else:
            H.bn_bwd_apply(x, G, a, bsh, mean, rstd, gamma, s[2], s[2], dx, False)
        return (dx,) + _defer((gamma, None, weight), (dgamma, dbeta, dW)) + (None, None, None, None, None)


class DenseBlockFn(torch.autograd.Function):

    @staticmethod
    def forward(ctx, x, bns, training, *params):
        L = len(bns)
        x = x if x.stride(3) == 1 else x.contiguous()
        B, Hh, Ww, c0 = x.shape
        growth = [params[3 * i + 2].shape[0] for i in range(L)]
        buf = empty((B, Hh, Ww, c0 + sum(growth)), x.device)
        H.masked_add(buf[..., :c0], src=x)
        ws = [params[3 * i + 2].contiguous() for i in range(L)]
        packs = H.conv_pack_many([(w, 0) for w in ws] + [(w, 1) for w in ws])
        stats, use_batch, c = [], [], c0
        for i in range(L):
            gamma, beta, weight = params[3 * i:3 * i + 3]
            bn = bns[i]
            xin = buf[..., :c]
            use_batch.append(bool(training) or not bn.track_running_stats)
            if use_batch[-1]:
                mean, rstd, a, bsh = bn_batch_stats(xin, bn)
            else:
                mean = bn.running_mean
                rstd = torch.rsqrt(bn.running_var + bn.eps)
                a = gamma.detach() * rstd
                bsh = beta.detach() - mean * a
            H.conv_fwd([xin], packs[i], growth[i], 3, 1, [buf[..., c:c + growth[i]]], in_scale=a, in_shift=bsh, relu_in=True)
            stats.append((mean, rstd, a, bsh))
            c += growth[i]
        ctx.meta = (L, c0, growth, use_batch)
        ctx.stats = stats
        ctx.packs_t = packs[L:]
        ctx.save_for_backward(buf, *params)
        return buf

    @staticmethod
    def backward(ctx, dout):
        L, c0, growth, use_batch = ctx.meta
        if ctx.stats is None:
            raise RuntimeError("DenseBlockFn: the per-layer statistics were released by a previous backward pass "
                               "(a second backward through the same graph is not supported)")
        buf = ctx.saved_tensors[0]
        params = ctx.saved_tensors[1:]
        B, Hh, Ww, Ct = buf.shape
        n = B * Hh * Ww
        dbuf = dout.contiguous().clone()
        grads = [None] * (3 * L)
        c = Ct
        for i in range(L - 1, -1, -1):
            gamma, beta, weight = params[3 * i:3 * i + 3]
            mean, rstd, a, bsh = ctx.stats[i]
            g = growth[i]
            c -= g
            xin, dy = buf[..., :c], dbuf[..., c:c + g]
            dW = zeros_like(weight)
            H.conv_wgrad([xin], dy, dW, None, 3, 1, in_scale=a, in_shift=bsh, relu_in=True)
            G = empty((B, Hh, Ww, c), buf.device)
            H.conv_fwd([dy], ctx.packs_t[i], c, 3, 1, [G])
            s = zeros((3, c), buf.device)
            H.chan_reduce(xin, G, a, bsh, mean, rstd, s[0], s[1], 1)
            if use_batch[i]:
                H.bn_bwd_apply(xin, G, a, bsh, mean, rstd, gamma, s[0], s[1], dbuf[..., :c], True, divisor=n)
            else:
                H.bn_bwd_apply(xin, G, a, bsh, mean, rstd, gamma, s[2], s[2], dbuf[..., :c], True)
            grads[3 * i:3 * i + 3] = [s[1], s[0], dW]
        ctx.stats = None
        ctx.packs_t = None
        return (dbuf[..., :c0], None, None) + _defer(params, grads)


def bn_batch_stats(x, bn):
    B, Hh, Ww, C = x.shape
    n = B * Hh * Ww
    out = torch.empty((5, C), device=x.device)
    track = bn.track_running_stats
    mom = bn.momentum if bn.momentum is not None else 0.1
    with torch.no_grad():
        acc64 = zeros((4 * C,), x.device).view(torch.float64)
        H.chan_moments(x, acc64)
        nbt = bn.num_batches_tracked if (track and bn.num_batches_tracked is not None and bn.num_batches_tracked.device == x.device) else None
        H.bn_finalize64(acc64, bn.weight.detach(), bn.bias.detach(), bn.running_mean if track else None,
                        bn.running_var if track else None, out, n, bn.eps, mom, counter=nbt)
        if nbt is not None:
            track = False
        if track and bn.num_batches_tracked is not None:
            bn.num_batches_tracked += 1
    return out[0], out[2], out[3], out[4]


def batch_moments(x):
    B, Hh, Ww, C = x.shape
    n = B * Hh * Ww
    s0 = zeros(C, x.device)
    s1 = zeros(C, x.device)
    H.chan_reduce(x, None, None, None, None, None, s0, s1, 0)
    mean = s0 / n
    s0b = zeros(C, x.device)
    s1b = zeros(C, x.device)
    H.chan_reduce(x, None, mean, None, None, None, s0b, s1b, 0)
    return mean, s1b / n, n


class AffineFn(torch.autograd.Function):

    @staticmethod
    def forward(ctx, hh, x, reverse):
        x = x if x.stride(3) == 1 else x.contiguous()
        hh = hh.contiguous()
        B, Hh, Ww, C = x.shape
        ch = C // 2
        y = empty((B, Hh, Ww, C), x.device)
        H.masked_add(y[..., :ch], src=x[..., :ch])
        r = empty((B, Hh, Ww, ch), x.device)
        logdet = zeros(B, x.device)
        H.affine_apply(hh, x[..., ch:], y[..., ch:], r, logdet, reverse)
        ctx.reverse = reverse
        ctx.save_for_backward(r, x if reverse else y)
        return y, logdet

    @staticmethod
    def backward(ctx, dy, dld):
        r, ref = ctx.saved_tensors
        dy = dy.contiguous()
        B, Hh, Ww, C = dy.shape
        ch = C // 2
        dx = torch.empty_like(dy)
        H.masked_add(dx[..., :ch], src=dy[..., :ch])
        dhh = empty((B, Hh, Ww, C), dy.device)
        g = dld.contiguous() if dld is not None else None
        H.affine_bwd(dy[..., ch:], ref[..., ch:], r, g, dx[..., ch:], dhh, ctx.reverse)
        return dhh, dx, None


class LSTMPointwiseFn(torch.autograd.Function):

    @staticmethod
    def forward(ctx, gates, c_prev):
        acts = gates.contiguous()
        B, Hh, Ww, R4 = acts.shape
        R = R4 // 4
        if c_prev is not None and c_prev.stride(3) != 1:
            c_prev = c_prev.contiguous()
        c_next = empty((B, Hh, Ww, R), acts.device)
        h_next = empty((B, Hh, Ww, R), acts.device)
        H.lstm_pointwise_fwd(acts, c_prev, c_next, h_next)
        ctx.has_c = c_prev is not None
        ctx.save_for_backward(acts, c_prev, c_next)
        return h_next, c_next

    @staticmethod
    def backward(ctx, dh, dc):
        acts, c_prev, c_next = ctx.saved_tensors
        dg = acts.clone()
        dc_prev = torch.empty_like(c_next)
        H.lstm_pointwise_bwd(dg, c_prev, c_next, dh.contiguous() if dh is not None else None,
                             dc.contiguous() if dc is not None else None, dc_prev)
        return dg, (dc_prev if ctx.has_c else None)


class ConvLSTMCellFn(torch.autograd.Function):

    @staticmethod
    def forward(ctx, weight, bias, h_cur, c_cur, *inputs):
        inputs = tuple(t if t.stride(3) == 1 else t.contiguous() for t in inputs)
        h_cur = h_cur if h_cur.stride(3) == 1 else h_cur.contiguous()
        if c_cur is not None and c_cur.stride(3) != 1:
            c_cur = c_cur.contiguous()
        B, Hh, Ww, _ = inputs[0].shape
        R4 = weight.shape[0]
        R = R4 // 4
        dev = weight.device
        gates = empty((B, Hh, Ww, R4), dev)
        segs = list(inputs) + [h_cur]
        H.conv3x3_auto(segs, weight, R4, [gates], bias=bias)
        c_next = empty((B, Hh, Ww, R), dev)
        h_next = empty((B, Hh, Ww, R), dev)
        H.lstm_pointwise_fwd(gates, c_cur, c_next, h_next)
        ctx.n_in = len(inputs)
        ctx.has_c = c_cur is not None
        ctx.consumed = False
        ctx.save_for_backward(weight, bias, h_cur, c_cur, gates, c_next, *inputs)
        ctx.set_materialize_grads(False)
        return h_next, c_next

    @staticmethod
    def backward(ctx, dh, dc):
        if ctx.consumed:
            raise RuntimeError("ConvLSTMCellFn: the gate buffer was consumed by a previous backward pass")
        ctx.consumed = True
        weight, bias, h_cur, c_cur, acts, c_next = ctx.saved_tensors[:6]
        inputs = ctx.saved_tensors[6:]
        dc_prev = torch.empty_like(c_next) if (ctx.has_c and ctx.needs_input_grad[3]) else None
        H.lstm_pointwise_bwd(acts, c_cur, c_next, dh.contiguous() if dh is not None else None,
                             dc.contiguous() if dc is not None else None, dc_prev)
        dg = acts
        segs = list(inputs) + [h_cur]
        dW = zeros_like(weight)
        db = zeros_like(bias)
        nrest = sum(t.shape[3] for t in segs[:-1])
        if h_cur.shape[3] == 64 and 32 < nrest <= 48 and nrest % 4 == 0 and H.wino_wgrad_eligible(nrest, weight.shape[0]):
            Cin = nrest + 64
            H.conv_wgrad(segs[:-1], dg, dW, db, 3, 1, cin_dst=Cin, cin_valid=nrest, ci_off0=0)
            H.conv_wgrad([h_cur], dg, dW, None, 3, 1, cin_dst=Cin, cin_valid=64, ci_off0=nrest)
        else:
            H.conv_wgrad(segs, dg, dW, db, 3, 1)
        need = [ctx.needs_input_grad[4 + i] for i in range(ctx.n_in)] + [ctx.needs_input_grad[2]]
        last = max([i for i, n in enumerate(need) if n], default=-1)
        dins = [None] * len(segs)
        if last >= 0:
            nch = sum(t.shape[3] for t in segs[:last + 1])
            dins[:last + 1] = [empty(t.shape, t.device) for t in segs[:last + 1]]
            H.conv3x3_auto([dg], weight, nch, dins[:last + 1], dgrad=True, nvalid=nch)
        return _defer((weight, bias), (dW, db)) + (dins[-1], dc_prev if ctx.has_c else None) + tuple(dins[:-1])


class GaussLogpFn(torch.autograd.Function):

    @staticmethod
    def forward(ctx, hz, z2, clip_mean, limits, want_eps):
        hz = hz.contiguous()
        z2 = z2 if z2.stride(3) == 1 else z2.contiguous()
        B = z2.shape[0]
        logp = zeros(B, z2.device)
        eps = empty(z2.shape, z2.device) if want_eps else None
        H.gauss_fwd(hz, z2, eps, logp, 0, clip_mean, limits)
        ctx.cfg = (clip_mean, limits)
        ctx.save_for_backward(hz, z2)
        ctx.mark_non_differentiable(*([eps] if want_eps else []))
        return logp, eps

    @staticmethod
    def backward(ctx, g, _geps):
        hz, z2 = ctx.saved_tensors
        clip_mean, limits = ctx.cfg
        dz2 = empty(z2.shape, z2.device)
        dhz = torch.empty_like(hz)
        H.gauss_bwd(hz, z2, None, g.contiguous(), dz2, dhz, 0, clip_mean, limits)
        return dhz, dz2, None, None, None


class GaussSampleFn(torch.autograd.Function):

    @staticmethod
    def forward(ctx, hz, eps, clip_mean, limits):
        hz = hz.contiguous()
        eps = eps.contiguous()
        B = eps.shape[0]
        logp = zeros(B, eps.device)
        z2 = empty(eps.shape, eps.device)
        H.gauss_fwd(hz, eps, z2, logp, 1, clip_mean, limits)
        ctx.cfg = (clip_mean, limits)
        ctx.save_for_backward(hz, eps)
        return z2, logp

    @staticmethod
    def backward(ctx, dz2, g):
        hz, eps = ctx.saved_tensors
        clip_mean, limits = ctx.cfg
        dhz = torch.empty_like(hz)
        H.gauss_bwd(hz, eps, dz2.contiguous() if dz2 is not None else None, g.contiguous() if g is not None else None, None, dhz, 1,
                    clip_mean, limits)
        return dhz, None, None, None


def latent_nonce(device):
    return torch.empty(2, dtype=torch.int64, device=device).random_()


def latent_nonces(device, k):
    return torch.empty((int(k), 2), dtype=torch.int64, device=device).random_()


class GaussDrawFn(torch.autograd.Function):

    @staticmethod
    def forward(ctx, hz, z1, eps, rng, clip_mean, limits):
        hz = hz if hz.stride(3) == 1 else hz.contiguous()
        B, Hh, Ww, C2 = hz.shape
        Ch = C2 // 2
        dev = hz.device
        if z1 is not None and z1.stride(3) != 1:
            z1 = z1.contiguous()
        out = empty((B, Hh, Ww, 2 * Ch if z1 is not None else Ch), dev)
        logp = zeros(B, dev)
        if eps is not None:
            eps = eps if eps.stride(3) == 1 else eps.contiguous()
# ... 126 lines not shown
        H.checker(dy, dx, not ctx.to_small)
        return dx, None


class PadHalvesFn(torch.autograd.Function):

    @staticmethod
    def forward(ctx, x, ch, pad, to_padded):
        x = x if x.stride(3) == 1 else x.contiguous()
        B, Hh, Ww, _ = x.shape
        y = empty((B, Hh, Ww, 2 * (ch + pad) if to_padded else 2 * ch), x.device)
        H.pad_halves(x, y, ch, pad, to_padded)
        ctx.cfg = (ch, pad, to_padded)
        return y

    @staticmethod
    def backward(ctx, dy):
        ch, pad, to_padded = ctx.cfg
        dy = dy if dy.stride(3) == 1 else dy.contiguous()
        B, Hh, Ww, _ = dy.shape
        dx = empty((B, Hh, Ww, 2 * ch if to_padded else 2 * (ch + pad)), dy.device)
        H.pad_halves(dy, dx, ch, pad, not to_padded)
        return dx, None, None, None


class UpsampleFn(torch.autograd.Function):

    @staticmethod
    def forward(ctx, x, scale):
        x = x.contiguous()
        B, Hh, Ww, C = x.shape
        ho, wo = int(math.floor(Hh * scale)), int(math.floor(Ww * scale))
        y = empty((B, ho, wo, C), x.device)
        H.upsample_fwd(x, y)
        ctx.in_shape = (B, Hh, Ww, C)
        return y

    @staticmethod
    def backward(ctx, dy):
        dx = empty(ctx.in_shape, dy.device)
        H.upsample_bwd(dy.contiguous(), dx)
        return dx, None


class CouplingTailFn(torch.autograd.Function):

    @staticmethod
    def forward(ctx, x, aux, w1, w2, wz, bz, kappa, reverse, mode):
        x = x if x.stride(3) == 1 else x.contiguous()
        aux = aux if aux.stride(3) == 1 else aux.contiguous()
        B, Hh, Ww, C = x.shape
        ch = C // 2
        dev = x.device
        nn_in = [x[..., :ch], aux] if mode == 0 else [aux]
        cin = sum(t.shape[3] for t in nn_in)
        w1, w2, wz = w1.contiguous(), w2.contiguous(), wz.contiguous()
        D = empty((B, Hh, Ww, 4), dev)
        H.c1_fwd(nn_in, w1, D[..., 0:1], relu_in=True, fill4=True)
        H.c1_fwd(nn_in + [D], w2, D[..., 1:2], relu_in=True, w_rows=cin + 1)
        hh = empty((B, Hh, Ww, C), dev)
        H.conv_fwd(nn_in + [D], H.conv_pack(wz, 0, cin + 4), C, 3, 1, [hh], bias=bz, kappa=kappa, relu_in=True, pad_rep=True)
        y = empty((B, Hh, Ww, C), dev)
        r = empty((B, Hh, Ww, ch), dev)
        logdet = zeros(B, dev)
        H.affine_apply(hh, x[..., ch:], y[..., ch:], r, logdet, reverse, x1=x[..., :ch], y1=y[..., :ch])
        ctx.reverse, ctx.mode, ctx.cin = reverse, mode, cin
        ctx.save_for_backward(x, aux, D, r, y, w1, w2, wz, bz, kappa)
        return y, logdet

    @staticmethod
    def backward(ctx, dy, dld):
        x, aux, D, r, y, w1, w2, wz, bz, kappa = ctx.saved_tensors
        reverse, mode, cin = ctx.reverse, ctx.mode, ctx.cin
        dy = dy.contiguous()
        B, Hh, Ww, C = dy.shape
        ch = C // 2
        dev = dy.device
        nn_in = [x[..., :ch], aux] if mode == 0 else [aux]
        dx = empty((B, Hh, Ww, C), dev)
        dhh = empty((B, Hh, Ww, C), dev)
        g = dld.contiguous() if dld is not None else None
        H.affine_bwd(dy[..., ch:], (x if reverse else y)[..., ch:], r, g, dx[..., ch:], dhh, reverse)
        dw1, dw2, dwz, dbz, dk = carve(dev, (1, cin, 3, 3), (1, cin + 1, 3, 3), (C, cin + 2, 3, 3), (C,), kappa.shape)
        H.conv_wgrad(nn_in + [D], dhh, dwz, dbz, 3, 1, kappa=kappa, relu_in=True, pad_rep=True, cin_dst=cin + 2)
        H.dkappa(wz, dwz, bz, dbz, kappa, dk)
        G = [empty(t.shape, dev) for t in nn_in]
        GD = empty((B, Hh, Ww, 4), dev)
        wz_t = H.conv_pack(wz, 1, cin + 4)
        H.conv_fwd([dhh], wz_t, cin + 4, 3, 1, G + [GD], kappa=kappa)
        H.conv_rep_border_fix(dhh, wz_t, G + [GD], kappa=kappa)
        if mode == 0:
            H.dense2_bwd(nn_in + [D], w1, w2, dw1, dw2, GD, D, G, [dx[..., :ch], G[1]], cin, add0=dy[..., :ch], rows1=cin, rows2=cin + 1)
            daux = G[1]
        else:
            H.dense2_bwd(nn_in + [D], w1, w2, dw1, dw2, GD, D, G, [G[0]], cin, rows1=cin, rows2=cin + 1)
            H.masked_add(dx[..., :ch], src=dy[..., :ch])
            daux = G[0]
        return (dx, daux) + _defer((w1, w2, wz, bz, kappa), (dw1, dw2, dwz, dbz, dk)) + (None, None)


_MIX_PRECISION = "f16" if os.environ.get("TMG_MIX_F16") else "f32"


def set_mix_precision(kind):
    global _MIX_PRECISION
    if kind not in ("f32", "f16"):
        raise ValueError("mix precision must be 'f32' or 'f16', got %r" % (kind,))
    _MIX_PRECISION = kind


def mix_precision():
    return _MIX_PRECISION


_RECOMPUTE = [bool(os.environ.get("TMG_RECOMPUTE"))]


def set_recompute(on):
    _RECOMPUTE[0] = bool(on)


def recompute():
    return _RECOMPUTE[0]


def set_winograd_precision(kind):
    H.set_winograd_precision(kind)


def winograd_precision():
    return H.winograd_precision()


def _mix16_ok(C):
    return _MIX_PRECISION == "f16" and C % 4 == 0 and C <= 256


def _mix_fwd(x, Wk, bk, packed=None):
    C = Wk.shape[0]
    y = empty(x.shape, x.device)
    if _mix16_ok(C):
        H.mix_f16(x, Wk.contiguous(), bk, y)
        return y
    if x.stride(3) == 1 and H.mix_f32(x, Wk.contiguous(), bk, y):
        return y
    H.conv_fwd([x], packed if packed is not None else H.conv_pack(Wk.reshape(C, C, 1, 1), 0), C, 1, 1, [y], bias=bk)
    return y


class MixFn(torch.autograd.Function):

    @staticmethod
    def forward(ctx, x, W, b):
        x = x if x.stride(3) == 1 else x.contiguous()
        ctx.save_for_backward(x, W)
        ctx.has_b = b is not None
        return _mix_fwd(x, W.detach(), b.detach() if b is not None else None)

    @staticmethod
    def backward(ctx, dy):
        x, W = ctx.saved_tensors
        dy = dy.contiguous()
        C = W.shape[0]
        dW = zeros_like(W)
        db = zeros(C, W.device)
        dx = _mix_bwd(x, dy, W, dW, db)
        return dx, dW, (db if ctx.has_b else None)
# ... 252 lines not shown
    def _activations(L, R, saved, k):
        if R is not None:
            return LevelCouplingFn._rebuild(L, R, k)
        acts, saved[k] = saved[k], None
        return acts

    @staticmethod
    def _grouped_wgrads(L, S):
        NL, C, ch = L.NL, L.C, L.ch
        if not H.conv_wgrad_grouped(S.wg_in, S.DH, C, S.dWz, S.dBz, 3, 1, **S.zc_kw):
            for k in range(NL):
                LevelCouplingFn._zero_conv_wgrad(L, S, k, S.wg_in[k], now=True)
        tmpX = zeros((NL, 4, ch + 4, 3, 3), S.DH.device)
        if not H.conv_wgrad_grouped(S.wg_in, S.DD, 2, tmpX, None, 3, 1, relu_in=True):
            for k in range(NL):
                H.conv_wgrad(S.wg_in[k], S.DD[..., 2 * k:2 * k + 2], tmpX[k][:2], None, 3, 1, relu_in=True)
        S.wg_in.clear()
        gdy = [g_ for _, g_ in S.mix_wg]
        if any(not torch.is_tensor(g_) for g_ in gdy):
            gdy = [H._halves(g_) for g_ in gdy]
        if not H.conv_wgrad_grouped([a for a, _ in S.mix_wg], None, C, S.dWm.view(NL, C, C, 1, 1), S.dbm, 1, 1, group_dy=gdy):
            for k in range(NL):
                LevelCouplingFn._mix_wgrad(L, S, k, *S.mix_wg[k], now=True)
        S.mix_wg.clear()
        return tmpX

    @staticmethod
    def _cond_bwd(L, S, cond, Wcat):
        NL, NLp, C, ch, Cc, cin = L[:6]
        dev = cond.device
        Gc = empty(cond.shape, dev)
        H.conv3x3_auto([S.DH, S.DD], Wcat, Cc, [Gc], dgrad=True)
        H.conv_rep_border_fix(S.DH, H.conv_pack(Wcat[:NL * C], 1), [Gc])
        H.masked_add(Gc, src=Gc, ref=cond)
        H.conv_wgrad([cond], S.DH, S.dWz, None, 3, 1, relu_in=True, pad_rep=True, cin_dst=cin + 2, cin_valid=Cc, ci_off0=ch)
        tmpC = zeros((NLp, 2, Cc, 3, 3), dev)
        H.conv_wgrad([cond], S.DD, tmpC.view(2 * NLp, Cc, 3, 3), None, 3, 1, relu_in=True)
        return Gc, tmpC

    @staticmethod
    def _finish(L, S, Wz, Bz, Kp, tmpX, tmpC):
        dK = empty(L.NL, Kp.device)
        H.level_finish(Wz, S.dWz, Bz, S.dBz, Kp, tmpX, tmpC, S.dW1, S.dW2, dK, zeros(4 * L.NL, Kp.device), L.ch, L.Cc)
        return dK

    @staticmethod
    def backward(ctx, dy, dld):
        L = ctx.level
        NL, NLp, C, ch, Cc, cin = L[:6]
        cond, Wm, bm, Wz, Wcat, Bz, Kp = ctx.saved_tensors[:7]
        wts = ctx.saved_tensors[7:]
        saved = ctx.saved
        if saved is None:
            raise RuntimeError("LevelCouplingFn: the saved activations were released by a previous backward pass "
                               "(a second backward through the same graph is not supported)")
        ctx.saved = None
        dy = dy.contiguous()
        bhw, dev = dy.shape[:3], dy.device
        g = dld.contiguous() if dld is not None else None
        dWz, dW1, dW2, dBz, dWm, dbm = carve(dev, (NL, C, cin + 2, 3, 3), (NL, 1, cin, 3, 3), (NL, 1, cin + 1, 3, 3), (NL, C), (NL, C, C),
                                             (NL, C))
        DH = empty(bhw + (NL * C,), dev)
        DD = empty(bhw + (2 * NLp,), dev)
        quad_last = NLp - NL == 1
        if NLp - NL > 1:
            DD[..., 2 * NL:].zero_()
        grouped = NL > 1 and ch + 4 <= 132
        PZt = H.conv_pack_batched(Wz, 1, ch + 4, (ch + 2, ch, Cc))
        PMt = H.conv_pack_batched(Wm.reshape(NL, C, C, 1, 1), 1)
        zc_kw = dict(relu_in=True, pad_rep=True, cin_dst=cin + 2, cin_valid=ch + 2, ci_split=ch, ci_off0=0, ci_off1=Cc)
        S = _LevelBwd(g, Wm, PZt, PMt, DH, DD, quad_last, grouped, zc_kw, [None] * NL, [None] * NL if grouped else None, dWz, dBz, dW1, dW2,
                      dWm, dbm)
        R = None
        if ctx.rec_out is not None:
            Hc_r, Dc_r, dc_of_r = LevelCouplingFn._cond_parts(L, cond, Wcat)
            Winv, binv = H.mat_inverse(Wm, bm)
            R = [Hc_r, dc_of_r, Winv, binv, zeros(bhw[0], dev), ctx.rec_out]
        ctx.rec_out = None
        if not L.fuse:
            step = LevelCouplingFn._bwd_wide
        else:
            step = LevelCouplingFn._bwd_fused_generative if L.reverse else LevelCouplingFn._bwd_fused_density
        dcur = dy
        for k in (range(NL) if L.reverse else range(NL - 1, -1, -1)):
            dcur = step(L, S, k, dcur, *LevelCouplingFn._activations(L, R, saved, k))
        tmpX = LevelCouplingFn._grouped_wgrads(L, S) if grouped else None
        Gc, tmpC = LevelCouplingFn._cond_bwd(L, S, cond, Wcat)
        dK = LevelCouplingFn._finish(L, S, Wz, Bz, Kp, tmpX, tmpC)
        grads = []
        for k in range(NL):
            grads += [dW1[k], dW2[k], dWz[k], dBz[k], dK[k].reshape(L.kps[k].shape)]
        return (dcur, Gc, dWm, dbm, None) + _defer(wts, grads)


class LevelMixFoldFn(torch.autograd.Function):

    @staticmethod
    def forward(ctx, meta, *params):
        tab, sign_s, perm, iperm, reverse, sgn, hw, K, C = meta
        dev = sign_s.device
        W = torch.empty((K, C, C), device=dev, dtype=torch.float64)
        Wm = empty((K, C, C), dev)
        bm = empty((K, C), dev)
        ld = empty(1, dev)
        H.lu_fold_fwd(tab, sign_s, perm, iperm, W, Wm, bm, ld, reverse, sgn, hw)
        ctx.meta = meta
        ctx.shapes = [t.shape if t is not None else None for t in params]
        ctx.save_for_backward(W, *[t for t in params if t is not None])
        ctx.set_materialize_grads(False)
        return Wm, bm, ld, Wm[:K - 1], bm[:K - 1], Wm[K - 1], bm[K - 1]

    @staticmethod
    def backward(ctx, dWm, dbm, dld, dWh, dbh, dWt, dbt):
        tab, sign_s, perm, iperm, reverse, sgn, hw, K, C = ctx.meta
        W = ctx.saved_tensors[0]
        dev = W.device
        dl = empty((K, C, C), dev)
        du = empty((K, C, C), dev)
        dlogs = empty((K, C), dev)
        da = empty((K, C), dev)
        db = empty((K, C), dev)
        split = dWm is None and dbm is None and dWt is not None and (dWh is not None or K == 1) and (dbt is None) == (dbh is None or K == 1)
        if split:
            dWm, dbm, dWt, dbt = (None if t is None else t.contiguous() for t in (dWh, dbh, dWt, dbt))
        else:
            full = zeros((K, C, C), dev) if dWm is None else dWm.clone()
            fb = zeros((K, C), dev) if dbm is None else dbm.clone()
            if dWh is not None:
                full[:K - 1] += dWh
            if dWt is not None:
                full[K - 1] += dWt
            if dbh is not None:
                fb[:K - 1] += dbh
            if dbt is not None:
                fb[K - 1] += dbt
            dWm, dbm, dWt, dbt = full, fb, None, None
        H.lu_fold_bwd(tab, sign_s, perm, iperm, W, dWm, dbm, dld.contiguous() if dld is not None else None, dl, du, dlogs, da, db,
                      reverse, sgn, hw, dWm_tail=dWt, dbm_tail=dbt)
        grads = []
        for k in range(K):
            sh = ctx.shapes[5 * k:5 * k + 5]
            grads += [dl[k], du[k], dlogs[k].view(sh[2]), da[k].view(sh[3]) if sh[3] is not None else None,
                      db[k].view(sh[4]) if sh[4] is not None else None]
        live = iter(ctx.saved_tensors[1:])
        params = [next(live) if sh is not None else None for sh in ctx.shapes]
        return (None,) + _defer(params, grads)


class LeadingChannelsFn(torch.autograd.Function):

    @staticmethod
    def forward(ctx, x, n):
        ctx.n, ctx.C = n, x.shape[3]
        ctx.set_materialize_grads(False)
        return x.view(x.shape), x[..., :n]

    @staticmethod
    def backward(ctx, dx, d1):
        if d1 is None:
            return dx, None
        if dx is None:
            dx = torch.zeros(d1.shape[:3] + (ctx.C,), device=d1.device, dtype=d1.dtype)
        dx[..., :ctx.n] += d1
        return dx, None


class EnsembleStats:

    def __init__(self, members, B, C, Hh, Ww, steps, device, out_mu, out_std, u=None, grid=None):
        if not (2 <= C <= 4):
# ... 812 lines not shown
```

include/tmglow_hip.h:

```cpp
#ifndef TMGLOW_HIP_H
#define TMGLOW_HIP_H
#include <stdint.h>

#ifdef __cplusplus
extern "C" {
#endif

#ifndef TMG_MAX_IN_SEG
#define TMG_MAX_IN_SEG 3
#define TMG_MAX_OUT_SEG 3
#endif

typedef struct ihipStream_t* tmg_stream_t;


int tmg_conv_pack(const void* w, void* wpk, int64_t Cout, int64_t Cin, int64_t cin_eff, int64_t ksize, int64_t mode,
                  tmg_stream_t st);

int tmg_conv_pack_map(const void* w, void* wpk, int64_t Cout, int64_t Cin, int64_t cin_eff, int64_t ksize, int64_t mode,
                      const int64_t* map, tmg_stream_t st);

int tmg_conv_fwd(const void* const* in_ptrs, const int64_t* in_desc, int64_t nseg, const void* wpk, const void* bias,
                 const void* kappa, const void* in_scale, const void* in_shift, void* const* out_ptrs,
                 const int64_t* out_desc, int64_t nout, const int64_t* dims, tmg_stream_t st);
// ... 116 lines not shown
int tmg_coupling_fwd(const void* x, void* out, void* rsave, void* y2save, const void* D, const void* hc, const void* wz,
                     const void* bz, const void* kappa, const void* Wm, const void* bm, void* logdet, const int64_t* dims,
                     tmg_stream_t st);

int tmg_coupling_bwd(const void* dout, const void* x, const void* r, const void* g, const void* Wm, const void* wz, const void* kappa,
                     void* DH, void* dtin, void* G0, void* GD, const int64_t* dims, tmg_stream_t st);

int tmg_coupling_fwd_halves(const void* x1, const void* x2, void* out1, void* out2, void* rsave, void* y2save, const void* D,
                            const void* hc, const void* wz, const void* bz, const void* kappa, const void* Wm, const void* bm,
                            void* logdet, const int64_t* dims, tmg_stream_t st);
int tmg_coupling_bwd_halves(const void* dout1, const void* dout2, const void* x2, const void* r, const void* g, const void* Wm,
                            const void* wz, const void* kappa, void* DH, void* dtin1, void* dtin2, void* G0, void* GD,
                            const int64_t* dims, tmg_stream_t st);


int tmg_mix_f16(const void* x, const int64_t* x_d, const void* W, const void* bias, void* y, const int64_t* y_d, const int64_t* dims,
                tmg_stream_t st);
int tmg_mat_inverse(const void* W, const void* b, void* Winv, void* binv, const int64_t* dims, tmg_stream_t st);
int tmg_adam_step(const void* tab, const void* chunks, const int64_t* dims, const float* fl, tmg_stream_t st);

int tmg_lu_fold_fwd(const void* tab, const void* sign_s, const void* perm, const void* iperm, void* W, void* Wm, void* bm, void* ld,
                    const int64_t* dims, const float* fl, tmg_stream_t st);
int tmg_lu_fold_bwd(const void* tab, const void* sign_s, const void* perm, const void* iperm, const void* W, const void* dWm, const void* dbm,
                    const void* dld, void* dl, void* du, void* dlogs, void* da, void* db, const int64_t* dims, const float* fl, tmg_stream_t st);
int tmg_lu_fold_bwd_split(const void* tab, const void* sign_s, const void* perm, const void* iperm, const void* W, const void* dWm,
                          const void* dbm, const void* dWm_tail, const void* dbm_tail, const void* dld, void* dl, void* du, void* dlogs,
                          void* da, void* db, const int64_t* dims, const float* fl, tmg_stream_t st);

int tmg_conv_wgrad_thin_grouped(const void* gtab, int64_t G, const int64_t* seg_channels, int64_t nseg, const void* dy, int64_t dy_stride,
                                void* dW, const int64_t* dims, tmg_stream_t st);

int tmg_mix_wgrad_grouped(const void* gtab, int64_t G, void* dW, void* db, const int64_t* dims, tmg_stream_t st);

int tmg_layer_planes(const void* src, void* dst, int64_t npix, int64_t CP, tmg_stream_t st);

int tmg_level_finish(const void* Wz, const void* dWz, const void* Bz, const void* dBz, const void* Kp, const void* tmpX, const void* tmpC,
                     void* dW1, void* dW2, void* dK, void* ws, const int64_t* dims, tmg_stream_t st);

int tmg_mix_f32(const void* x, const int64_t* x_d, const void* W, const void* bias, void* y, const int64_t* y_d,
                const int64_t* dims, tmg_stream_t st);
int tmg_mix_f32_affine_fwd(const void* x, const int64_t* x_d, const void* hh, const int64_t* hh_d, const void* W, const void* bias,
                           void* y, const int64_t* y_d, void* r, void* y2, void* logdet, const int64_t* dims, tmg_stream_t st);
int tmg_mix_f32_affine_bwd(const void* dy, const int64_t* dy_d, const void* W, const void* r, const void* t2, const int64_t* t2_d,
                           const void* g, const void* kappa, void* dto1, void* dtin2, const int64_t* dtin2_d, void* dhh,
                           const int64_t* dhh_d, const int64_t* dims, tmg_stream_t st);


#define TMG_SUM_TERMS_MAX 8

int tmg_gauss_sample(const void* hz, const int64_t* hz_d, const void* eps_in, const int64_t* ei_d, const void* pass,
                     const int64_t* p_d, void* out, const int64_t* o_d, int64_t pass_off, void* eps_out, void* logp, const void* nonce,
                     const int64_t* dims, const float* fl, tmg_stream_t st);
int tmg_gauss_sample_keyed(const void* hz, const int64_t* hz_d, const void* eps_in, const int64_t* ei_d, const void* pass,
                           const int64_t* p_d, void* out, const int64_t* o_d, int64_t pass_off, void* eps_out, void* logp,
                           const void* keys, const int64_t* dims, const float* fl, tmg_stream_t st);

int tmg_ens_accum(const void* y, const int64_t* y_d, const void* u, const void* out_mu, const void* out_std, void* smean, void* sm2,
                  void* tmean, void* tm2, void* mean_out, void* std_out, void* mag_mean, void* mag_std, const int64_t* o_d,
                  const int64_t* dims, tmg_stream_t st);
int tmg_ens_time_finalize(const void* tmean, const void* tm2, void* tm_mean, void* tm_std, void* rms_mean, void* rms_std,
                          const int64_t* dims, tmg_stream_t st);
int tmg_ens_turb_accum(const void* y, const int64_t* y_d, const void* u, const void* out_mu, const void* out_std, const void* tmean,
                       void* vmean, void* vm2, void* cuv, void* tvort, void* vort_mean, void* vort_std, const int64_t* dims,
                       const float* fl, tmg_stream_t st);
int tmg_ens_turb_finalize(const void* tm2, const void* cuv, const void* tvort, void* uv_mean, void* uv_std, void* tke_mean,
                          void* tke_std, void* tv_mean, void* tv_std, const int64_t* dims, tmg_stream_t st);

int tmg_ens_score_store(const void* y, const int64_t* y_d, void* xs, const int64_t* dims, tmg_stream_t st);
int tmg_ens_score_step(const void* xs, const void* target, const int64_t* t_d, const void* scale, void* crps, void* crps_fair,
                       void* hist, void* tcrps, void* tcrps_fair, const int64_t* o_d, const int64_t* dims, tmg_stream_t st);

int tmg_spec_rows(const void* y, const int64_t* y_d, const void* u, const void* out_mu, const void* out_std, const void* ft, void* yw,
                  const int64_t* dims, tmg_stream_t st);
int tmg_spec_cols(const void* ft, const void* yw, const void* perm, const void* offs, void* part, const int64_t* dims, const float* fl,
                  tmg_stream_t st);
int tmg_spec_accum(const void* part, void* smean, void* sm2, void* tmean, void* mean_out, void* std_out, const int64_t* dims,
                   tmg_stream_t st);
int tmg_spec_finalize(const void* tmean, void* tm_mean, void* tm_std, const int64_t* dims, tmg_stream_t st);

#include "tmglow_hip_tspec.h"
#include "tmglow_hip_quant.h"
#include "tmglow_hip_gram.h"
#include "tmglow_hip_sfun.h"

int tmg_reverse_loss_fwd(const void* y, const void* ld, void* loss, const int64_t* dims, const float* fl, tmg_stream_t st);
int tmg_reverse_loss_bwd(const void* y, const void* g, void* dy, void* dld, const int64_t* dims, const float* fl, tmg_stream_t st);

int tmg_sum_terms(const void* const* terms, const int64_t* lens, int64_t n, void* out, int64_t B, tmg_stream_t st);
int tmg_vec_sum(const void* g, int64_t B, void* out, tmg_stream_t st);

int tmg_level_pack(const void* tab, void* Wz, void* Wcat, void* Bz, void* Kp, const int64_t* dims, tmg_stream_t st);

int tmg_spread2(const void* dy, const int64_t* dy_d, void* up, const int64_t* dims, tmg_stream_t st);


int tmg_phys_fwd(const void* y, const void* target, void* sums, void* pstar_out, void* ustar_out, const int64_t* dims,
                 const float* fl, tmg_stream_t st);
int tmg_phys_fields(const void* u, const void* p, void* ustar, void* pstar, const int64_t* dims, const float* fl, tmg_stream_t st);
int tmg_phys_fields_bwd(const void* u, const void* p, const void* gustar, const void* gpstar, void* du, void* dp, const int64_t* dims,
                        const float* fl, tmg_stream_t st);
int tmg_phys_rms(const void* y, const void* trms, void* mean_out, void* coef_out, void* sum_out, const int64_t* dims,
                 tmg_stream_t st);
int tmg_phys_bwd(const void* y, const void* target, const void* mean, const void* coef, void* dy, const int64_t* dims,
                 const float* fl, tmg_stream_t st);
int tmg_phys_bwd_dev(const void* y, const void* target, const void* mean, const void* coef, void* dy, const void* upstream,
                     const int64_t* dims, const float* fl, tmg_stream_t st);

#ifdef __cplusplus
}
#endif
#endif
```

Baseline: 1518 samples/s.

## Batch deferred wgrad reduce launches into one multi-job fold kernel per backward scope

Weight-gradient workspace reductions (direct and Winograd) are no longer launched right after each wgrad partial kernel. Each one is recorded as a job descriptor in a Python fold queue, and the queue is flushed as a single grouped kernel that dispatches blocks to jobs by a start-offset table. The goal is fewer small kernel launches and better GPU fill during backward. In exchange, each job needs its own workspace that stays live until the flush, which raises memory use, and a linear job search runs per block.

```diff
diff --git a/deep-turbulence_amd/csrc/tmg_common.h b/deep-turbulence_amd/csrc/tmg_common.h
--- a/deep-turbulence_amd/csrc/tmg_common.h
+++ b/deep-turbulence_amd/csrc/tmg_common.h
@@ -16,6 +16,13 @@
 
 #define TMG_MAX_IN_SEG 3
 #define TMG_MAX_OUT_SEG 3
+
+#define TMG_FOLD_JOB_N 24
+#define TMG_FOLD_JOBS 24
+#define TMG_FOLD_NONE (-1)
+#define TMG_FOLD_DIRECT 0
+#define TMG_FOLD_WINO 1
+int tmg_wino_fold_many(const int64_t* jobs, int64_t njobs, hipStream_t st);
 
 struct TmgSeg {
     const float* p;
diff --git a/deep-turbulence_amd/csrc/tmg_conv.hip b/deep-turbulence_amd/csrc/tmg_conv.hip
--- a/deep-turbulence_amd/csrc/tmg_conv.hip
+++ b/deep-turbulence_amd/csrc/tmg_conv.hip
@@ -914,14 +914,14 @@
     if (do_bias && tid < NCO * 16 && co0 + tid < p.Cout) atomicAdd(p.dbias + co0 + tid, bsum * osc);
 }
 
-__global__ void conv_wgrad_reduce_kernel(const float* __restrict__ ws, float* __restrict__ dW, float* __restrict__ dbias,
-                                         const float* __restrict__ kappa, int gx, int gy, int gz, int NP, int NCO, int PPG,
-                                         int pairs_total, int Cin, int Cout, int ntaps, int xchunk, int cin_valid, int ci_split,
-                                         int ci_off0, int ci_off1, int ksplit, int bpg, long long dw_gstride, int db_gstride) {
+__device__ __forceinline__ void conv_wgrad_reduce_body(int bx, int by, const float* __restrict__ ws, float* __restrict__ dW, float* __restrict__ dbias,
+                                                       const float* __restrict__ kappa, int gx, int gy, int gz, int NP, int NCO, int PPG,
+                                                       int pairs_total, int Cin, int Cout, int ntaps, int xchunk, int cin_valid, int ci_split,
+                                                       int ci_off0, int ci_off1, int ksplit, int bpg, long long dw_gstride, int db_gstride) {
     const int nws = ksplit ? 1 : 4;
     const int items = gy * gz * nws * NP * NCO * 64;
-    const int i = blockIdx.x * blockDim.x + threadIdx.x;
-    const int x0 = blockIdx.y * xchunk, x1 = min(gx, x0 + xchunk);
+    const int i = bx * blockDim.x + threadIdx.x;
+    const int x0 = by * xchunk, x1 = min(gx, x0 + xchunk);
     const float osc = out_scale_of(kappa);
     if (i < items) {
         int r_ = i;
@@ -978,6 +978,30 @@
             atomicAdd(dbias + co, a * osc);
         }
     }
+}
+
+__global__ void conv_wgrad_reduce_kernel(const float* __restrict__ ws, float* __restrict__ dW, float* __restrict__ dbias,
+                                         const float* __restrict__ kappa, int gx, int gy, int gz, int NP, int NCO, int PPG,
+                                         int pairs_total, int Cin, int Cout, int ntaps, int xchunk, int cin_valid, int ci_split,
+                                         int ci_off0, int ci_off1, int ksplit, int bpg, long long dw_gstride, int db_gstride) {
+    conv_wgrad_reduce_body(blockIdx.x, blockIdx.y, ws, dW, dbias, kappa, gx, gy, gz, NP, NCO, PPG, pairs_total, Cin, Cout, ntaps, xchunk,
+                           cin_valid, ci_split, ci_off0, ci_off1, ksplit, bpg, dw_gstride, db_gstride);
+}
+
+struct FoldJob {
+    const float* ws; float* dW; float* dbias; const float* kappa;
+    long long dw_gstride;
+    int gx, gy, gz, NP, NCO, PPG, pairs_total, Cin, Cout, ntaps, xchunk, cin_valid, ci_split, ci_off0, ci_off1, ksplit, bpg, db_gstride, nbx;
+};
+struct FoldJobs { FoldJob j[TMG_FOLD_JOBS]; int start[TMG_FOLD_JOBS + 1]; int njobs; };
+
+__global__ void conv_wgrad_fold_many_kernel(FoldJobs J) {
+    int job = 0;
+    while (job + 1 < J.njobs && (int)blockIdx.x >= J.start[job + 1]) ++job;
+    const FoldJob& f = J.j[job];
+    const int b = (int)blockIdx.x - J.start[job];
+    conv_wgrad_reduce_body(b % f.nbx, b / f.nbx, f.ws, f.dW, f.dbias, f.kappa, f.gx, f.gy, f.gz, f.NP, f.NCO, f.PPG, f.pairs_total, f.Cin, f.Cout,
+                           f.ntaps, f.xchunk, f.cin_valid, f.ci_split, f.ci_off0, f.ci_off1, f.ksplit, f.bpg, f.dw_gstride, f.db_gstride);
 }
 
 __global__ void conv_pack_kernel(const float* __restrict__ w, float* __restrict__ wpk, int Cout, int Cin, int ntaps,
@@ -1720,7 +1744,8 @@
 static int wgrad_impl(const void* const* in_ptrs, const int64_t* in_desc, int64_t nseg, const void* in_scale,
                       const void* in_shift, const void* dy, const int64_t* dy_desc, void* dW, void* dbias,
                       const void* kappa, void* ws, int64_t ws_floats, const int64_t* dims, hipStream_t st,
-                      const long long* gtab, int ngroups, int dy_goff, long long dw_gstride, int db_gstride, int64_t* plan = nullptr) {
+                      const long long* gtab, int ngroups, int dy_goff, long long dw_gstride, int db_gstride, int64_t* plan = nullptr,
+                      int64_t* job = nullptr) {
     WgradP p;
     p.nseg = (int)nseg;
     p.vec4 = tmg_decode_in(p.in, in_ptrs, in_desc, nseg).vec4;
@@ -1772,7 +1797,14 @@
     TMG_WG_CASE(9, 1) TMG_WG_CASE(9, 2)
 #undef TMG_WG_CASE
     if (lrc != 0 || plan) return lrc;
-    if (p.ws) {
+    if (job) job[0] = TMG_FOLD_NONE;
+    if (p.ws && job) {
+        const int64_t v[TMG_FOLD_JOB_N] = {TMG_FOLD_DIRECT, (int64_t)(uintptr_t)p.ws, (int64_t)(uintptr_t)p.dW, (int64_t)(uintptr_t)p.dbias,
+                                           (int64_t)(uintptr_t)p.kappa, pl.gx, pl.gy, pl.gz, pl.NP, pl.NCO, pl.PPG,
+                                           (p.Cin_pad >> 4) * p.ksize * p.ksize, p.cin_dst, p.Cout, p.ksize * p.ksize, 32, p.cin_valid, p.ci_split,
+                                           p.ci_off0, p.ci_off1, pl.ksplit, bpg, dw_gstride, db_gstride};
+        for (int i = 0; i < TMG_FOLD_JOB_N; ++i) job[i] = v[i];
+    } else if (p.ws) {
         const int items = pl.gy * pl.gz * (pl.ksplit ? 1 : 4) * pl.NP * pl.NCO * 64;
         int xchunk = 32;
         const int xc = (pl.gx + xchunk - 1) / xchunk;
@@ -1788,6 +1820,14 @@
                               const void* in_shift, const void* dy, const int64_t* dy_desc, void* dW, void* dbias,
                               const void* kappa, void* ws, int64_t ws_floats, const int64_t* dims, hipStream_t st) {
     return wgrad_impl(in_ptrs, in_desc, nseg, in_scale, in_shift, dy, dy_desc, dW, dbias, kappa, ws, ws_floats, dims, st, nullptr, 1, 0, 0, 0);
+}
+
+extern "C" int tmg_conv_wgrad_job(const void* const* in_ptrs, const int64_t* in_desc, int64_t nseg, const void* in_scale,
+                                  const void* in_shift, const void* dy, const int64_t* dy_desc, void* dW, void* dbias,
+                                  const void* kappa, void* ws, int64_t ws_floats, const int64_t* dims, hipStream_t st, int64_t* job) {
+    if (!job) return -3;
+    return wgrad_impl(in_ptrs, in_desc, nseg, in_scale, in_shift, dy, dy_desc, dW, dbias, kappa, ws, ws_floats, dims, st, nullptr, 1, 0, 0, 0,
+                      nullptr, job);
 }
 
 extern "C" int tmg_conv_wgrad_plan(const void* const* in_ptrs, const int64_t* in_desc, int64_t nseg, const void* in_scale,
@@ -1806,6 +1846,61 @@
     if (ngroups < 1 || !gtab) return -3;
     return wgrad_impl(in_ptrs, in_desc, nseg, nullptr, nullptr, dy, dy_desc, dW, dbias, nullptr, ws, ws_floats, dims, st,
                       (const long long*)gtab, (int)ngroups, (int)gdims[0], (long long)gdims[1], (int)gdims[2]);
+}
+
+extern "C" int tmg_conv_wgrad_grouped_job(const void* const* in_ptrs, const int64_t* in_desc, int64_t nseg, const void* gtab,
+                                          int64_t ngroups, const int64_t* gdims, const void* dy, const int64_t* dy_desc, void* dW,
+                                          void* dbias, void* ws, int64_t ws_floats, const int64_t* dims, hipStream_t st, int64_t* job) {
+    if (ngroups < 1 || !gtab || !job) return -3;
+    return wgrad_impl(in_ptrs, in_desc, nseg, nullptr, nullptr, dy, dy_desc, dW, dbias, nullptr, ws, ws_floats, dims, st,
+                      (const long long*)gtab, (int)ngroups, (int)gdims[0], (long long)gdims[1], (int)gdims[2], nullptr, job);
+}
+
+extern "C" int tmg_wgrad_fold_many(const int64_t* jobs, int64_t njobs, hipStream_t st) {
+    if (njobs < 0 || (njobs > 0 && !jobs)) return -3;
+    FoldJobs J;
+    int n = 0, nwino = 0;
+    long long blocks = 0;
+    auto launch = [&]() -> int {
+        if (n == 0) return 0;
+        J.njobs = n;
+        J.start[n] = (int)blocks;
+        for (int k = n + 1; k <= TMG_FOLD_JOBS; ++k) J.start[k] = (int)blocks;
+        hipLaunchKernelGGL(conv_wgrad_fold_many_kernel, dim3((unsigned)blocks), dim3(256), 0, st, J);
+        TMG_CHECK_LAUNCH();
+        n = 0; blocks = 0;
+        return 0;
+    };
+    for (int64_t k = 0; k < njobs; ++k) {
+        const int64_t* v = jobs + k * TMG_FOLD_JOB_N;
+        if (v[0] == TMG_FOLD_NONE) continue;
+        if (v[0] == TMG_FOLD_WINO) { ++nwino; continue; }
+        if (v[0] != TMG_FOLD_DIRECT) return -3;
+        FoldJob f;
+        f.ws = (const float*)(uintptr_t)v[1]; f.dW = (float*)(uintptr_t)v[2]; f.dbias = (float*)(uintptr_t)v[3]; f.kappa = (const float*)(uintptr_t)v[4];
+        f.gx = (int)v[5]; f.gy = (int)v[6]; f.gz = (int)v[7]; f.NP = (int)v[8]; f.NCO = (int)v[9]; f.PPG = (int)v[10]; f.pairs_total = (int)v[11];
+        f.Cin = (int)v[12]; f.Cout = (int)v[13]; f.ntaps = (int)v[14]; f.xchunk = (int)v[15]; f.cin_valid = (int)v[16]; f.ci_split = (int)v[17];
+        f.ci_off0 = (int)v[18]; f.ci_off1 = (int)v[19]; f.ksplit = (int)v[20]; f.bpg = (int)v[21]; f.dw_gstride = (long long)v[22];
+        f.db_gstride = (int)v[23];
+        if (!f.ws || !f.dW || f.gx < 1 || f.gy < 1 || f.gz < 1 || f.NP < 1 || f.NP > 9 || f.NCO < 1 || f.NCO > 4 || f.xchunk < 1 || f.bpg < 1 ||
+            f.ntaps < 1 || f.PPG < 1 || f.Cin < 1 || f.Cout < 1)
+            return -3;
+        const long long items = (long long)f.gy * f.gz * (f.ksplit ? 1 : 4) * f.NP * f.NCO * 64;
+        const long long nbx = (items + 255) / 256, xc = (f.gx + f.xchunk - 1) / f.xchunk;
+        if (nbx * xc >= (1LL << 30)) return -3;
+        f.nbx = (int)nbx;
+        if (n == TMG_FOLD_JOBS || blocks + nbx * xc >= (1LL << 31)) {
+            const int rc = launch();
+            if (rc != 0) return rc;
+        }
+        J.j[n] = f;
+        J.start[n] = (int)blocks;
+        blocks += nbx * xc;
+        ++n;
+    }
+    const int rc = launch();
+    if (rc != 0) return rc;
+    return nwino ? tmg_wino_fold_many(jobs, njobs, st) : 0;
 }
 
 extern "C" int64_t tmg_conv_wgrad_grouped_ws_floats(const int64_t* dims, int64_t ngroups) {
diff --git a/deep-turbulence_amd/csrc/tmg_wino.hip b/deep-turbulence_amd/csrc/tmg_wino.hip
--- a/deep-turbulence_amd/csrc/tmg_wino.hip
+++ b/deep-turbulence_amd/csrc/tmg_wino.hip
@@ -1468,14 +1468,13 @@
 }
 
 template <int NG>
-__global__ __launch_bounds__(64 * NG) TMG_PACKED_F32 void wino_wgrad_reduce_kernel(const float* __restrict__ ws, float* __restrict__ dW, float* __restrict__ dbias,
-                                                                   int gx, int gy, int gz, int CIT, int NCO, int Cin, int Cout, int cin_dst,
-                                                                   int cin_valid, int ci_split, int ci_off0, int ci_off1, int bpg,
-                                                                   long long dw_gstride, int db_gstride) {
-    extern __shared__ __attribute__((aligned(16))) float red_[];
+__device__ __forceinline__ TMG_PACKED_F32 void wino_wgrad_reduce_body(int blk, float* red_, const float* __restrict__ ws, float* __restrict__ dW,
+                                                                       float* __restrict__ dbias, int gx, int gy, int gz, int CIT, int NCO, int Cin,
+                                                                       int Cout, int cin_dst, int cin_valid, int ci_split, int ci_off0, int ci_off1,
+                                                                       int bpg, long long dw_gstride, int db_gstride) {
     float (*red)[64][37] = reinterpret_cast<float (*)[64][37]>(red_);
     const int lane = threadIdx.x & 63, grp = threadIdx.x >> 6;
-    int r_ = blockIdx.x;
+    int r_ = blk;
     const int n = r_ % NCO; r_ /= NCO;
     const int i = r_ % CIT; r_ /= CIT;
     const int bz = r_ % gz, by = r_ / gz;
@@ -1552,6 +1551,33 @@
             dbias[co] += s_;
         }
     }
+}
+
+template <int NG>
+__global__ __launch_bounds__(64 * NG) TMG_PACKED_F32 void wino_wgrad_reduce_kernel(const float* __restrict__ ws, float* __restrict__ dW, float* __restrict__ dbias,
+                                                                   int gx, int gy, int gz, int CIT, int NCO, int Cin, int Cout, int cin_dst,
+                                                                   int cin_valid, int ci_split, int ci_off0, int ci_off1, int bpg,
+                                                                   long long dw_gstride, int db_gstride) {
+    extern __shared__ __attribute__((aligned(16))) float red_[];
+    wino_wgrad_reduce_body<NG>(blockIdx.x, red_, ws, dW, dbias, gx, gy, gz, CIT, NCO, Cin, Cout, cin_dst, cin_valid, ci_split, ci_off0, ci_off1,
+                               bpg, dw_gstride, db_gstride);
+}
+
+struct WinoFoldJob {
+    const float* ws; float* dW; float* dbias;
+    long long dw_gstride;
+    int gx, gy, gz, CIT, NCO, Cin, Cout, cin_dst, cin_valid, ci_split, ci_off0, ci_off1, bpg, db_gstride;
+};
+struct WinoFoldJobs { WinoFoldJob j[TMG_FOLD_JOBS]; int start[TMG_FOLD_JOBS + 1]; int njobs; };
+
+template <int NG>
+__global__ __launch_bounds__(64 * NG) TMG_PACKED_F32 void wino_wgrad_fold_many_kernel(WinoFoldJobs J) {
+    extern __shared__ __attribute__((aligned(16))) float red_[];
+    int job = 0;
+    while (job + 1 < J.njobs && (int)blockIdx.x >= J.start[job + 1]) ++job;
+    const WinoFoldJob& f = J.j[job];
+    wino_wgrad_reduce_body<NG>((int)blockIdx.x - J.start[job], red_, f.ws, f.dW, f.dbias, f.gx, f.gy, f.gz, f.CIT, f.NCO, f.Cin, f.Cout, f.cin_dst,
+                               f.cin_valid, f.ci_split, f.ci_off0, f.ci_off1, f.bpg, f.dw_gstride, f.db_gstride);
 }
 
 struct WinoWPlan { int CIT, NCO, gx, gy, gz; size_t ws_floats; };
@@ -1605,7 +1631,8 @@
 
 static int wino_wgrad_impl(const void* const* in_ptrs, const int64_t* in_desc, int64_t nseg, const void* dy, const int64_t* dy_desc,
                            void* dW, void* dbias, void* ws, int64_t ws_floats, const int64_t* dims, hipStream_t st, const long long* gtab,
-                           int ngroups, int dy_goff, long long dw_gstride, int db_gstride, int64_t* plan = nullptr) {
+                           int ngroups, int dy_goff, long long dw_gstride, int db_gstride, int64_t* plan = nullptr, int64_t* job = nullptr) {
+    if (job) job[0] = TMG_FOLD_NONE;
     WinoWP p;
     p.nseg = (int)nseg;
     if (p.nseg < 1 || p.nseg > TMG_MAX_IN_SEG) return -3;
@@ -1637,6 +1664,13 @@
 #undef TMG_WW_CASE
     if (rc != 0 || plan) return rc;
     const int ng = wino_wgrad_reduce_groups(pl.gx);
+    if (job) {
+        const int64_t v[TMG_FOLD_JOB_N] = {TMG_FOLD_WINO, (int64_t)(uintptr_t)p.ws, (int64_t)(uintptr_t)dW, (int64_t)(uintptr_t)dbias, 0,
+                                           pl.gx, pl.gy, pl.gz, pl.CIT, pl.NCO, p.Cin, p.Cout, cin_dst, cin_valid, ci_split, ci_off0, ci_off1,
+                                           p.bpg, dw_gstride, db_gstride, ng, 0, 0, 0};
+        for (int i = 0; i < TMG_FOLD_JOB_N; ++i) job[i] = v[i];
+        return 0;
+    }
     if (ng == 16) {
         TMG_LDS_OPTIN((&wino_wgrad_reduce_kernel<16>));
         hipLaunchKernelGGL(wino_wgrad_reduce_kernel<16>, dim3(pl.gy * pl.gz * pl.CIT * pl.NCO), dim3(1024), 15 * 64 * 37 * sizeof(float), st,
@@ -1669,6 +1703,70 @@
                            (int)gdims[0], (long long)gdims[1], (int)gdims[2]);
 }
 
+extern "C" int tmg_conv_wino_wgrad_job(const void* const* in_ptrs, const int64_t* in_desc, int64_t nseg, const void* dy, const int64_t* dy_desc,
+                                       void* dW, void* dbias, void* ws, int64_t ws_floats, const int64_t* dims, hipStream_t st, int64_t* job) {
+    if (!job) return -3;
+    return wino_wgrad_impl(in_ptrs, in_desc, nseg, dy, dy_desc, dW, dbias, ws, ws_floats, dims, st, nullptr, 1, 0, 0, 0, nullptr, job);
+}
+
+extern "C" int tmg_conv_wino_wgrad_grouped_job(const void* const* in_ptrs, const int64_t* in_desc, int64_t nseg, const void* gtab,
+                                               int64_t ngroups, const int64_t* gdims, const void* dy, const int64_t* dy_desc, void* dW,
+                                               void* dbias, void* ws, int64_t ws_floats, const int64_t* dims, hipStream_t st, int64_t* job) {
+    if (ngroups < 1 || !gtab || !job) return -3;
+    return wino_wgrad_impl(in_ptrs, in_desc, nseg, dy, dy_desc, dW, dbias, ws, ws_floats, dims, st, (const long long*)gtab, (int)ngroups,
+                           (int)gdims[0], (long long)gdims[1], (int)gdims[2], nullptr, job);
+}
+
+template <int NG>
+static int wino_fold_many_ng(const int64_t* jobs, int64_t njobs, hipStream_t st) {
+    WinoFoldJobs J;
+    int n = 0;
+    long long blocks = 0;
+    auto launch = [&]() -> int {
+        if (n == 0) return 0;
+        J.njobs = n;
+        for (int k = n; k <= TMG_FOLD_JOBS; ++k) J.start[k] = (int)blocks;
+        TMG_LDS_OPTIN((&wino_wgrad_fold_many_kernel<NG>));
+        hipLaunchKernelGGL(wino_wgrad_fold_many_kernel<NG>, dim3((unsigned)blocks), dim3(64 * NG), (NG - 1) * 64 * 37 * sizeof(float), st, J);
+        TMG_CHECK_LAUNCH();
+        n = 0; blocks = 0;
+        return 0;
+    };
+    for (int64_t k = 0; k < njobs; ++k) {
+        const int64_t* v = jobs + k * TMG_FOLD_JOB_N;
+        if (v[0] != TMG_FOLD_WINO || v[20] != NG) continue;
+        WinoFoldJob f;
+        f.ws = (const float*)(uintptr_t)v[1]; f.dW = (float*)(uintptr_t)v[2]; f.dbias = (float*)(uintptr_t)v[3];
+        f.gx = (int)v[5]; f.gy = (int)v[6]; f.gz = (int)v[7]; f.CIT = (int)v[8]; f.NCO = (int)v[9]; f.Cin = (int)v[10]; f.Cout = (int)v[11];
+        f.cin_dst = (int)v[12]; f.cin_valid = (int)v[13]; f.ci_split = (int)v[14]; f.ci_off0 = (int)v[15]; f.ci_off1 = (int)v[16];
+        f.bpg = (int)v[17]; f.dw_gstride = (long long)v[18]; f.db_gstride = (int)v[19];
+        const long long nb = (long long)f.gy * f.gz * f.CIT * f.NCO;
+        if (n == TMG_FOLD_JOBS || blocks + nb >= (1LL << 31)) {
+            const int rc = launch();
+            if (rc != 0) return rc;
+        }
+        J.j[n] = f;
+        J.start[n] = (int)blocks;
+        blocks += nb;
+        ++n;
+    }
+    return launch();
+}
+
+int tmg_wino_fold_many(const int64_t* jobs, int64_t njobs, hipStream_t st) {
+    for (int64_t k = 0; k < njobs; ++k) {
+        const int64_t* v = jobs + k * TMG_FOLD_JOB_N;
+        if (v[0] != TMG_FOLD_WINO) continue;
+        if (!v[1] || !v[2] || v[5] < 1 || v[6] < 1 || v[7] < 1 || v[6] * v[7] > (1 << 24) || v[8] < 2 || v[8] > 4 || v[9] < 2 || v[9] > 4 ||
+            v[17] < 1 || (v[20] != 4 && v[20] != 8 && v[20] != 16))
+            return -3;
+    }
+    int rc = wino_fold_many_ng<4>(jobs, njobs, st);
+    if (rc == 0) rc = wino_fold_many_ng<8>(jobs, njobs, st);
+    if (rc == 0) rc = wino_fold_many_ng<16>(jobs, njobs, st);
+    return rc;
+}
+
 extern "C" int tmg_conv_wino_wgrad_plan(const void* const* in_ptrs, const int64_t* in_desc, int64_t nseg, const void* dy, const int64_t* dy_desc,
                                         void* dW, void* dbias, void* ws, int64_t ws_floats, const int64_t* dims, hipStream_t st, int64_t ngroups,
                                         int64_t* plan) {
diff --git a/deep-turbulence_amd/tmg_hip.py b/deep-turbulence_amd/tmg_hip.py
--- a/deep-turbulence_amd/tmg_hip.py
+++ b/deep-turbulence_amd/tmg_hip.py
@@ -33,6 +33,8 @@
 QUANT_EXPORTS = ["tmg_ens_quant_step"]
 GRAM_EXPORTS = ["tmg_ens_gram_plan", "tmg_ens_gram_step", "tmg_ens_gram_traj"]
 SFUN_EXPORTS = ["tmg_ens_sfun_plan", "tmg_ens_sfun_step"]
+FOLD_EXPORTS = ["tmg_wgrad_fold_many", "tmg_conv_wgrad_job", "tmg_conv_wgrad_grouped_job", "tmg_conv_wino_wgrad_job",
+                "tmg_conv_wino_wgrad_grouped_job"]
 RET_I64 = ("tmg_conv_wgrad_ws_floats", "tmg_conv_wgrad_grouped_ws_floats", "tmg_conv_wino_wgrad_ws_floats",
            "tmg_conv_wino_wgrad_grouped_ws_floats")
 
@@ -42,7 +44,8 @@
     inc = os.path.join(os.path.dirname(_HERE), "include")
     headers = [os.path.join(CSRC, "tmg_common.h"), os.path.join(inc, "tmglow_hip.h"), os.path.join(inc, "tmglow_hip_plan.h"),
                os.path.join(inc, "tmglow_hip_tspec.h"), os.path.join(inc, "tmglow_hip_quant.h"),
-               os.path.join(inc, "tmglow_hip_gram.h"), os.path.join(inc, "tmglow_hip_sfun.h")]
+               os.path.join(inc, "tmglow_hip_gram.h"), os.path.join(inc, "tmglow_hip_sfun.h"),
+               os.path.join(inc, "tmglow_hip_fold.h")]
     hmt = max(os.path.getmtime(h) for h in headers)
     objdir = os.path.join(_HERE, "build")
     os.makedirs(objdir, exist_ok=True)
@@ -93,7 +96,7 @@
         for name in PLAN_EXPORTS:
             getattr(_lib, name).restype = ctypes.c_int
             getattr(_lib, name).argtypes = PLAN_ARGTYPES[name]
-        for name in TSPEC_EXPORTS + QUANT_EXPORTS + GRAM_EXPORTS + SFUN_EXPORTS:
+        for name in TSPEC_EXPORTS + QUANT_EXPORTS + GRAM_EXPORTS + SFUN_EXPORTS + FOLD_EXPORTS:
             getattr(_lib, name).restype = ctypes.c_int
     return _lib
 
@@ -412,6 +415,85 @@
     return buf
 
 
+FOLD_JOB_N = 24
+FOLD_JOBS = 24
+FOLD_ARENA_CAP = 1 << 27
+_ARENA = {}
+
+
+def wgrad_fold_many(jobs):
+    if jobs:
+        flat = [int(v) for j in jobs for v in j]
+        _chk(lib().tmg_wgrad_fold_many(_i64(*flat), c_i64(len(jobs)), _stream()), "tmg_wgrad_fold_many")
+
+
+class fold_queue:
+    active = None
+
+    def __init__(self, arena_cap=None):
+        self.cap = int(arena_cap) if arena_cap is not None else FOLD_ARENA_CAP
+        self.jobs, self.keep, self.used, self.launches = [], [], 0, 0
+        self.outer = None
+
+    def __enter__(self):
+        self.outer = fold_queue.active
+        if self.outer is None:
+            fold_queue.active = self
+        return self.outer or self
+
+    def __exit__(self, et, ev, tb):
+        q = self.outer or self
+        if self.outer is None:
+            fold_queue.active = None
+        if et is None:
+            q.flush()
+        else:
+            q.jobs, q.keep, q.used = [], [], 0
+        return False
+
+    def take(self, nfloats, device):
+        n = (max(int(nfloats), 1) + 63) & ~63
+        if torch.cuda.is_current_stream_capturing():
+            t = torch.empty(n, device=device, dtype=torch.float32)
+            self.keep.append(t)
+            return t
+        if self.used > 0 and self.used + n > self.cap:
+            self.flush()
+        key = (device.index, torch._C._cuda_getCurrentRawStream(torch._C._cuda_getDevice()))
+        buf = _ARENA.get(key)
+        if buf is None or buf.numel() < self.used + n:
+            if buf is not None:
+                self.keep.append(buf)
+            size = max(self.used + n, min(self.cap, 2 * buf.numel() if buf is not None else 1 << 22))
+            buf = torch.empty(size, device=device, dtype=torch.float32)
+            _ARENA[key] = buf
+            self.used = 0
+        out = buf[self.used:self.used + n]
+        self.used += n
+        return out
+
+    def push(self, job):
+        if job[0] >= 0:
+            self.jobs.append(list(job))
+
+    def flush(self):
+        if self.jobs:
+            wgrad_fold_many(self.jobs)
+            self.launches += 1
+        self.jobs, self.keep, self.used = [], [], 0
+
+
+def _wgrad_ws(nfloats, device):
+    q = fold_queue.active
+    return (q.take(nfloats, device) if q is not None else workspace(nfloats, device)), q
+
+
+def _job():
+    j = (c_i64 * FOLD_JOB_N)()
+    j[0] = -1
+    return j
+
+
 _WINO_WGRAD_CIN_MIN = 32
 _WINO_WGRAD_PIX_MIN = 1 << 20
 
@@ -427,7 +509,13 @@
             and conv_wino_wgrad(inputs, dy, dW, dbias, relu_in, pad_rep, cin_dst, cin_valid, ci_split, ci_off0, ci_off1)):
         return
     dims = _i64(B, Hin, Win, Hout, Wout, ksize, stride, Cin, Cout, relu_in, pad_rep, cin_dst, cin_valid, ci_split, ci_off0, ci_off1)
-    ws = workspace(lib().tmg_conv_wgrad_ws_floats(dims), dy.device) if use_ws else None
+    ws, q = _wgrad_ws(lib().tmg_conv_wgrad_ws_floats(dims), dy.device) if use_ws else (None, None)
+    if q is not None:
+        job = _job()
+        _chk(lib().tmg_conv_wgrad_job(ip, idesc, c_i64(n_in), _ptr(in_scale), _ptr(in_shift), _ptr(dy), _d2(dy), _ptr(dW), _ptr(dbias),
+                                      _ptr(kappa), _ptr(ws), c_i64(ws.numel()), dims, _stream(), job), "tmg_conv_wgrad_job")
+        q.push(job)
+        return
     _chk(lib().tmg_conv_wgrad(ip, idesc, c_i64(n_in), _ptr(in_scale), _ptr(in_shift), _ptr(dy), _d2(dy), _ptr(dW), _ptr(dbias),
                               _ptr(kappa), _ptr(ws), c_i64(ws.numel() if ws is not None else 0), dims, _stream()), "tmg_conv_wgrad")
 
@@ -444,7 +532,15 @@
     wd = _i64(B, Hin, Win, Cin, Cout, relu_in, pad_rep, cin_dst, cin_valid, ci_split, ci_off0, ci_off1)
     need = lib().tmg_conv_wino_wgrad_ws_floats(wd)
     if need > 0:
-        ws = workspace(need, dy.device)
+        ws, q = _wgrad_ws(need, dy.device)
+        if q is not None:
+            job = _job()
+            rc = lib().tmg_conv_wino_wgrad_job(ip, idesc, c_i64(n_in), _ptr(dy), _d2(dy), _ptr(dW), _ptr(dbias), _ptr(ws), c_i64(ws.numel()), wd,
+                                               _stream(), job)
+            if _launched(rc, "tmg_conv_wino_wgrad_job"):
+                q.push(job)
+                return True
+            return False
         rc = lib().tmg_conv_wino_wgrad(ip, idesc, c_i64(n_in), _ptr(dy), _d2(dy), _ptr(dW), _ptr(dbias), _ptr(ws), c_i64(ws.numel()), wd, _stream())
         if _launched(rc, "tmg_conv_wino_wgrad"):
             return True
@@ -555,11 +651,18 @@
         wd = _i64(B, Hin, Win, Cin, Cg, relu_in, pad_rep, cin_dst, cin_valid, ci_split, ci_off0, ci_off1)
         need = lib().tmg_conv_wino_wgrad_grouped_ws_floats(wd, c_i64(G))
         if need > 0:
-            ws = workspace(need, dy.device)
+            ws, q = _wgrad_ws(need, dy.device)
             gd = _i64(Cg, dW[0].numel(), dbias[0].numel() if dbias is not None else 0)
-            rc = lib().tmg_conv_wino_wgrad_grouped(ip, idesc, c_i64(n_in), _ptr(gtab), c_i64(G), gd, _ptr(dy), _d2(dy), _ptr(dW), _ptr(dbias),
-                                                   _ptr(ws), c_i64(ws.numel()), wd, _stream())
+            if q is not None:
+                job = _job()
+                rc = lib().tmg_conv_wino_wgrad_grouped_job(ip, idesc, c_i64(n_in), _ptr(gtab), c_i64(G), gd, _ptr(dy), _d2(dy), _ptr(dW),
+                                                           _ptr(dbias), _ptr(ws), c_i64(ws.numel()), wd, _stream(), job)
+            else:
+                rc = lib().tmg_conv_wino_wgrad_grouped(ip, idesc, c_i64(n_in), _ptr(gtab), c_i64(G), gd, _ptr(dy), _d2(dy), _ptr(dW), _ptr(dbias),
+                                                       _ptr(ws), c_i64(ws.numel()), wd, _stream())
             if _launched(rc, "tmg_conv_wino_wgrad_grouped"):
+                if q is not None:
+                    q.push(job)
                 return True
     if (group_dy is not None and ksize == 1 and stride == 1 and Cg == Cin and Cin in (16, 32) and cin_dst in (0, Cin)
             and cin_valid in (0, Cin) and ci_split == 0 and os.environ.get("TMG_NO_MIX_WGRAD_KERNEL") is None
@@ -579,8 +682,16 @@
         if _launched(rc, "tmg_conv_wgrad_thin_grouped"):
             return True
     dims = _i64(B, Hin, Win, Hout, Wout, ksize, stride, Cin, Cg, relu_in, pad_rep, cin_dst, cin_valid, ci_split, ci_off0, ci_off1)
-    ws = workspace(lib().tmg_conv_wgrad_grouped_ws_floats(dims, c_i64(G)), dy.device)
+    ws, q = _wgrad_ws(lib().tmg_conv_wgrad_grouped_ws_floats(dims, c_i64(G)), dy.device)
     gd = _i64(Cg, dW[0].numel(), dbias[0].numel() if dbias is not None else 0)
+    if q is not None:
+        job = _job()
+        rc = lib().tmg_conv_wgrad_grouped_job(ip, idesc, c_i64(n_in), _ptr(gtab), c_i64(G), gd, _ptr(dy), _d2(dy), _ptr(dW), _ptr(dbias),
+                                              _ptr(ws), c_i64(ws.numel()), dims, _stream(), job)
+        if not _launched(rc, "tmg_conv_wgrad_grouped_job"):
+            return False
+        q.push(job)
+        return True
     rc = lib().tmg_conv_wgrad_grouped(ip, idesc, c_i64(n_in), _ptr(gtab), c_i64(G), gd, _ptr(dy), _d2(dy), _ptr(dW), _ptr(dbias),
                                       _ptr(ws), c_i64(ws.numel()), dims, _stream())
     return _launched(rc, "tmg_conv_wgrad_grouped")
diff --git a/deep-turbulence_amd/tmg_ops.py b/deep-turbulence_amd/tmg_ops.py
--- a/deep-turbulence_amd/tmg_ops.py
+++ b/deep-turbulence_amd/tmg_ops.py
@@ -385,23 +385,24 @@
         dbuf = dout.contiguous().clone()
         grads = [None] * (3 * L)
         c = Ct
-        for i in range(L - 1, -1, -1):
-            gamma, beta, weight = params[3 * i:3 * i + 3]
-            mean, rstd, a, bsh = ctx.stats[i]
-            g = growth[i]
-            c -= g
-            xin, dy = buf[..., :c], dbuf[..., c:c + g]
-            dW = zeros_like(weight)
-            H.conv_wgrad([xin], dy, dW, None, 3, 1, in_scale=a, in_shift=bsh, relu_in=True)
-            G = empty((B, Hh, Ww, c), buf.device)
-            H.conv_fwd([dy], ctx.packs_t[i], c, 3, 1, [G])
-            s = zeros((3, c), buf.device)
-            H.chan_reduce(xin, G, a, bsh, mean, rstd, s[0], s[1], 1)
-            if use_batch[i]:
-                H.bn_bwd_apply(xin, G, a, bsh, mean, rstd, gamma, s[0], s[1], dbuf[..., :c], True, divisor=n)
-            else:
-                H.bn_bwd_apply(xin, G, a, bsh, mean, rstd, gamma, s[2], s[2], dbuf[..., :c], True)
-            grads[3 * i:3 * i + 3] = [s[1], s[0], dW]
+        with H.fold_queue():
+            for i in range(L - 1, -1, -1):
+                gamma, beta, weight = params[3 * i:3 * i + 3]
+                mean, rstd, a, bsh = ctx.stats[i]
+                g = growth[i]
+                c -= g
+                xin, dy = buf[..., :c], dbuf[..., c:c + g]
+                dW = zeros_like(weight)
+                H.conv_wgrad([xin], dy, dW, None, 3, 1, in_scale=a, in_shift=bsh, relu_in=True)
+                G = empty((B, Hh, Ww, c), buf.device)
+                H.conv_fwd([dy], ctx.packs_t[i], c, 3, 1, [G])
+                s = zeros((3, c), buf.device)
+                H.chan_reduce(xin, G, a, bsh, mean, rstd, s[0], s[1], 1)
+                if use_batch[i]:
+                    H.bn_bwd_apply(xin, G, a, bsh, mean, rstd, gamma, s[0], s[1], dbuf[..., :c], True, divisor=n)
+                else:
+                    H.bn_bwd_apply(xin, G, a, bsh, mean, rstd, gamma, s[2], s[2], dbuf[..., :c], True)
+                grads[3 * i:3 * i + 3] = [s[1], s[0], dW]
         ctx.stats = None
         ctx.packs_t = None
         return (dbuf[..., :c0], None, None) + _defer(params, grads)
@@ -538,8 +539,9 @@
         nrest = sum(t.shape[3] for t in segs[:-1])
         if h_cur.shape[3] == 64 and 32 < nrest <= 48 and nrest % 4 == 0 and H.wino_wgrad_eligible(nrest, weight.shape[0]):
             Cin = nrest + 64
-            H.conv_wgrad(segs[:-1], dg, dW, db, 3, 1, cin_dst=Cin, cin_valid=nrest, ci_off0=0)
-            H.conv_wgrad([h_cur], dg, dW, None, 3, 1, cin_dst=Cin, cin_valid=64, ci_off0=nrest)
+            with H.fold_queue():
+                H.conv_wgrad(segs[:-1], dg, dW, db, 3, 1, cin_dst=Cin, cin_valid=nrest, ci_off0=0)
+                H.conv_wgrad([h_cur], dg, dW, None, 3, 1, cin_dst=Cin, cin_valid=64, ci_off0=nrest)
         else:
             H.conv_wgrad(segs, dg, dW, db, 3, 1)
         need = [ctx.needs_input_grad[4 + i] for i in range(ctx.n_in)] + [ctx.needs_input_grad[2]]
@@ -832,7 +834,8 @@
         g = dld.contiguous() if dld is not None else None
         H.affine_bwd(dy[..., ch:], (x if reverse else y)[..., ch:], r, g, dx[..., ch:], dhh, reverse)
         dw1, dw2, dwz, dbz, dk = carve(dev, (1, cin, 3, 3), (1, cin + 1, 3, 3), (C, cin + 2, 3, 3), (C,), kappa.shape)
-        H.conv_wgrad(nn_in + [D], dhh, dwz, dbz, 3, 1, kappa=kappa, relu_in=True, pad_rep=True, cin_dst=cin + 2)
+        with H.fold_queue():
+            H.conv_wgrad(nn_in + [D], dhh, dwz, dbz, 3, 1, kappa=kappa, relu_in=True, pad_rep=True, cin_dst=cin + 2)
         H.dkappa(wz, dwz, bz, dbz, kappa, dk)
         G = [empty(t.shape, dev) for t in nn_in]
         GD = empty((B, Hh, Ww, 4), dev)
@@ -1251,10 +1254,11 @@
         else:
             step = LevelCouplingFn._bwd_fused_generative if L.reverse else LevelCouplingFn._bwd_fused_density
         dcur = dy
-        for k in (range(NL) if L.reverse else range(NL - 1, -1, -1)):
-            dcur = step(L, S, k, dcur, *LevelCouplingFn._activations(L, R, saved, k))
-        tmpX = LevelCouplingFn._grouped_wgrads(L, S) if grouped else None
-        Gc, tmpC = LevelCouplingFn._cond_bwd(L, S, cond, Wcat)
+        with H.fold_queue():
+            for k in (range(NL) if L.reverse else range(NL - 1, -1, -1)):
+                dcur = step(L, S, k, dcur, *LevelCouplingFn._activations(L, R, saved, k))
+            tmpX = LevelCouplingFn._grouped_wgrads(L, S) if grouped else None
+            Gc, tmpC = LevelCouplingFn._cond_bwd(L, S, cond, Wcat)
         dK = LevelCouplingFn._finish(L, S, Wz, Bz, Kp, tmpX, tmpC)
         grads = []
         for k in range(NL):
diff --git a/include/tmglow_hip.h b/include/tmglow_hip.h
--- a/include/tmglow_hip.h
+++ b/include/tmglow_hip.h
@@ -222,6 +222,7 @@
 #include "tmglow_hip_quant.h"
 #include "tmglow_hip_gram.h"
 #include "tmglow_hip_sfun.h"
+#include "tmglow_hip_fold.h"
 
 int tmg_reverse_loss_fwd(const void* y, const void* ld, void* loss, const int64_t* dims, const float* fl, tmg_stream_t st);
 int tmg_reverse_loss_bwd(const void* y, const void* g, void* dy, void* dld, const int64_t* dims, const float* fl, tmg_stream_t st);
diff --git a/include/tmglow_hip_fold.h b/include/tmglow_hip_fold.h
--- /dev/null
+++ b/include/tmglow_hip_fold.h
@@ -0,0 +1,19 @@
+#ifndef TMGLOW_HIP_FOLD_H
+#define TMGLOW_HIP_FOLD_H
+
+#define TMG_FOLD_JOB_N 24
+#define TMG_FOLD_JOBS 24
+int tmg_wgrad_fold_many(const int64_t* jobs, int64_t njobs, tmg_stream_t st);
+int tmg_conv_wgrad_job(const void* const* in_ptrs, const int64_t* in_desc, int64_t nseg, const void* in_scale,
+                       const void* in_shift, const void* dy, const int64_t* dy_desc, void* dW, void* dbias, const void* kappa,
+                       void* ws, int64_t ws_floats, const int64_t* dims, tmg_stream_t st, int64_t* job);
+int tmg_conv_wgrad_grouped_job(const void* const* in_ptrs, const int64_t* in_desc, int64_t nseg, const void* gtab, int64_t ngroups,
+                               const int64_t* gdims, const void* dy, const int64_t* dy_desc, void* dW, void* dbias, void* ws,
+                               int64_t ws_floats, const int64_t* dims, tmg_stream_t st, int64_t* job);
+int tmg_conv_wino_wgrad_job(const void* const* in_ptrs, const int64_t* in_desc, int64_t nseg, const void* dy, const int64_t* dy_desc,
+                            void* dW, void* dbias, void* ws, int64_t ws_floats, const int64_t* dims, tmg_stream_t st, int64_t* job);
+int tmg_conv_wino_wgrad_grouped_job(const void* const* in_ptrs, const int64_t* in_desc, int64_t nseg, const void* gtab, int64_t ngroups,
+                                    const int64_t* gdims, const void* dy, const int64_t* dy_desc, void* dW, void* dbias, void* ws,
+                                    int64_t ws_floats, const int64_t* dims, tmg_stream_t st, int64_t* job);
+
+#endif
```

After: 1511 samples/s, median of 2. About the same (-0.4%).
